# gpauloski/BERT-PyTorch

Measured on AMD Instinct MI355X. Metric: sequences/sec, higher is better.
Workload: dtype bf16; 1 GPU; model=bert_large_uncased_config (24L/1024H/16h, vocab 30528), phase=1, global_batch=768, named_global_batch=65536, seq_len=128, local_batch=96, accumulation=8, optimizer=FusedLAMB (HIP multi-tensor) + fp32 masters, weights=bf16 matmul weights + fp32 LN/bias (fp32 LAMB masters), parallelism=dp1

## Files before the change

### bert_pytorch_amd/models/bert.py

```python

from __future__ import annotations

import logging
import math
from typing import Optional

import torch
import torch.nn.functional as F
from torch import nn

from .. import ops
from ..config import BertConfig

logger = logging.getLogger(__name__)


def _autocast_dtype(ref: torch.Tensor) -> torch.dtype:
    if ref.is_cuda and torch.is_autocast_enabled():
        return torch.get_autocast_gpu_dtype()
    return ref.dtype


class LinearActivation(nn.Module):

    def __init__(self, in_features: int, out_features: int, act: str = "gelu"):
        super().__init__()
        self.in_features = in_features
        self.out_features = out_features
        self.act = act
        self.weight = nn.Parameter(torch.empty(out_features, in_features))
        self.bias = nn.Parameter(torch.empty(out_features))
        self.reset_parameters()

    def reset_parameters(self) -> None:
        nn.init.kaiming_uniform_(self.weight, a=math.sqrt(5))
        bound = 1 / math.sqrt(self.in_features)
        nn.init.uniform_(self.bias, -bound, bound)

    def forward(self, x: torch.Tensor) -> torch.Tensor:
        if self.act in ("gelu", "bias_gelu"):
            y = ops.linear_nobias(x, self.weight)
            return ops.fused_bias_gelu(y, self.bias)
        y = F.linear(x, self.weight, self.bias)
        if self.act in ("tanh", "bias_tanh"):
            return torch.tanh(y)
        if self.act == "relu":
            return F.relu(y)
        if self.act == "swish":
            return y * torch.sigmoid(y)
        raise ValueError(f"unsupported activation {self.act!r}")


class BertEmbeddings(nn.Module):

    def __init__(self, config: BertConfig):
        super().__init__()
        self.word_embeddings = nn.Embedding(config.vocab_size, config.hidden_size)
        self.position_embeddings = nn.Embedding(
            config.max_position_embeddings, config.hidden_size
        )
        if config.next_sentence:
            self.token_type_embeddings = nn.Embedding(
                config.type_vocab_size, config.hidden_size
            )
        else:
            self.token_type_embeddings = None
        self.LayerNorm = ops.FusedLayerNorm(config.hidden_size, eps=1e-12)
        self.dropout_prob = config.hidden_dropout_prob

    def forward(
        self, input_ids: torch.Tensor, token_type_ids: Optional[torch.Tensor]
    ) -> torch.Tensor:
        tok_w = (
            self.token_type_embeddings.weight
            if self.token_type_embeddings is not None
            else None
        )
        return ops.fused_embedding_ln_dropout(
            input_ids,
            token_type_ids if tok_w is not None else None,
            self.word_embeddings.weight,
            self.position_embeddings.weight,
            tok_w,
            self.LayerNorm.weight,
            self.LayerNorm.bias,
            self.dropout_prob,
            self.training,
        )


class _PackedQKV(nn.Module):

    def __init__(self, hidden_size: int):
        super().__init__()
        self.hidden_size = hidden_size
        self.qkv_weight = nn.Parameter(torch.empty(3 * hidden_size, hidden_size))
        self.qkv_bias = nn.Parameter(torch.zeros(3 * hidden_size))

    def forward(self, x: torch.Tensor) -> torch.Tensor:
        return ops.fused_linear(x, self.qkv_weight, self.qkv_bias)

    def _save_to_state_dict(self, destination, prefix, keep_vars):
        h = self.hidden_size
        w = self.qkv_weight if keep_vars else self.qkv_weight.detach()
        b = self.qkv_bias if keep_vars else self.qkv_bias.detach()
        for i, name in enumerate(("query", "key", "value")):
            destination[f"{prefix}{name}.weight"] = w[i * h : (i + 1) * h]
            destination[f"{prefix}{name}.bias"] = b[i * h : (i + 1) * h]

    def _load_from_state_dict(
        self, state_dict, prefix, local_metadata, strict,
        missing_keys, unexpected_keys, error_msgs,
    ):
        h = self.hidden_size
        parts_w, parts_b = [], []
        for name in ("query", "key", "value"):
            wk, bk = f"{prefix}{name}.weight", f"{prefix}{name}.bias"
            if wk in state_dict:
                parts_w.append(state_dict.pop(wk))
            elif strict:
                missing_keys.append(wk)
            if bk in state_dict:
                parts_b.append(state_dict.pop(bk))
            elif strict:
                missing_keys.append(bk)
        with torch.no_grad():
            if len(parts_w) == 3:
                self.qkv_weight.copy_(torch.cat([p.reshape(h, h) for p in parts_w], 0))
            if len(parts_b) == 3:
                self.qkv_bias.copy_(torch.cat([p.reshape(h) for p in parts_b], 0))


class BertSelfOutput(nn.Module):

    def __init__(self, config: BertConfig):
        super().__init__()
        self.dense = nn.Linear(config.hidden_size, config.hidden_size)
        self.LayerNorm = ops.FusedLayerNorm(config.hidden_size, eps=1e-12)
        self.dropout_prob = config.hidden_dropout_prob

    def forward(self, hidden: torch.Tensor, residual: torch.Tensor) -> torch.Tensor:
        y = ops.linear_nobias(hidden, self.dense.weight)
        return ops.fused_bias_dropout_residual_ln(
            y, self.dense.bias, residual,
            self.LayerNorm.weight, self.LayerNorm.bias,
            self.dropout_prob, self.training,
        )


class BertAttention(nn.Module):

    def __init__(self, config: BertConfig):
        super().__init__()
        if config.hidden_size % config.num_attention_heads != 0:
            raise ValueError(
                f"hidden_size {config.hidden_size} not divisible by "
                f"num_attention_heads {config.num_attention_heads}"
            )
        self.num_heads = config.num_attention_heads
        self.self = _PackedQKV(config.hidden_size)
        self.output = BertSelfOutput(config)
        self.dropout_prob = config.attention_probs_dropout_prob

    def forward(
        self, x: torch.Tensor, seqlens: torch.Tensor, max_seqlen: int = 0
    ) -> torch.Tensor:
        qkv = self.self(x)
        if max_seqlen:
            ctx = ops.fused_attention_varlen(
                qkv, seqlens, max_seqlen, self.num_heads,
                self.dropout_prob, self.training,
            )
        else:
            ctx = ops.fused_attention(
                qkv, seqlens, self.num_heads, self.dropout_prob, self.training
            )
        return self.output(ctx, x)


class BertIntermediate(nn.Module):
    def __init__(self, config: BertConfig):
        super().__init__()
        self.dense_act = LinearActivation(
            config.hidden_size, config.intermediate_size, act=config.hidden_act
        )

    def forward(self, x: torch.Tensor) -> torch.Tensor:
        return self.dense_act(x)


class BertOutput(nn.Module):
    def __init__(self, config: BertConfig):
        super().__init__()
        self.dense = nn.Linear(config.intermediate_size, config.hidden_size)
        self.LayerNorm = ops.FusedLayerNorm(config.hidden_size, eps=1e-12)
        self.dropout_prob = config.hidden_dropout_prob

    def forward(self, hidden: torch.Tensor, residual: torch.Tensor) -> torch.Tensor:
        y = ops.linear_nobias(hidden, self.dense.weight)
        return ops.fused_bias_dropout_residual_ln(
            y, self.dense.bias, residual,
            self.LayerNorm.weight, self.LayerNorm.bias,
            self.dropout_prob, self.training,
        )


class BertLayer(nn.Module):
    def __init__(self, config: BertConfig):
        super().__init__()
        self.attention = BertAttention(config)
        self.intermediate = BertIntermediate(config)
        self.output = BertOutput(config)
        self._ffn_gelu = config.hidden_act in ("gelu", "bias_gelu")

    def forward(
        self, x: torch.Tensor, seqlens: torch.Tensor, max_seqlen: int = 0
    ) -> torch.Tensor:
        attn = self.attention(x, seqlens, max_seqlen)
        if self._ffn_gelu and ops.ffn_supported(attn):
            y = ops.fused_ffn(
                attn,
                self.intermediate.dense_act.weight,
                self.intermediate.dense_act.bias,
                self.output.dense.weight,
            )
            return ops.fused_bias_dropout_residual_ln(
                y, self.output.dense.bias, attn,
                self.output.LayerNorm.weight, self.output.LayerNorm.bias,
                self.output.dropout_prob, self.training,
            )
        inter = self.intermediate(attn)
        return self.output(inter, attn)


class BertEncoder(nn.Module):

    def __init__(self, config: BertConfig):
        super().__init__()
        self.layer = nn.ModuleList(
            BertLayer(config) for _ in range(config.num_hidden_layers)
        )
        self.output_all_encoded_layers = config.output_all_encoded_layers
        self._checkpoint_activations = False

    def _checkpointed_forward(self, x, seqlens, max_seqlen=0):
        num_layers = len(self.layer)
        chunk = int(math.sqrt(num_layers)) or 1

        def run(start, end):
            def custom(hidden, lens):
                for layer in self.layer[start:end]:
                    hidden = layer(hidden, lens, max_seqlen)
                return hidden

            return custom

        for start in range(0, num_layers, chunk):
            end = min(start + chunk, num_layers)
            x = torch.utils.checkpoint.checkpoint(
                run(start, end), x, seqlens, use_reentrant=False
            )
        return x

    def forward(
        self, x: torch.Tensor, seqlens: torch.Tensor, max_seqlen: int = 0
    ):
        all_layers = []
        if self._checkpoint_activations:
            x = self._checkpointed_forward(x, seqlens, max_seqlen)
        else:
            for layer in self.layer:
                x = layer(x, seqlens, max_seqlen)
                if self.output_all_encoded_layers:
                    all_layers.append(x)
        if not self.output_all_encoded_layers or self._checkpoint_activations:
            all_layers.append(x)
        return all_layers


class BertPooler(nn.Module):
    def __init__(self, config: BertConfig):
        super().__init__()
        self.dense_act = LinearActivation(
            config.hidden_size, config.hidden_size, act="tanh"
        )

    def forward(self, hidden: torch.Tensor) -> torch.Tensor:
        return self.dense_act(hidden[:, 0])


class BertPredictionHeadTransform(nn.Module):
    def __init__(self, config: BertConfig):
        super().__init__()
        self.dense_act = LinearActivation(
            config.hidden_size, config.hidden_size, act=config.hidden_act
        )
        self.LayerNorm = ops.FusedLayerNorm(config.hidden_size, eps=1e-12)

    def forward(self, x: torch.Tensor) -> torch.Tensor:
        return self.LayerNorm(self.dense_act(x))


class BertLMPredictionHead(nn.Module):

    def __init__(self, config: BertConfig, embedding_weights: torch.Tensor):
        super().__init__()
        self.transform = BertPredictionHeadTransform(config)
        self.decoder = nn.Linear(
            embedding_weights.size(1), embedding_weights.size(0), bias=False
        )
        self.decoder.weight = embedding_weights
        self.bias = nn.Parameter(torch.zeros(embedding_weights.size(0)))

    def forward(self, x: torch.Tensor) -> torch.Tensor:
        x = self.transform(x)
        return F.linear(x, self.decoder.weight, self.bias)


class BertPreTrainingHeads(nn.Module):
    def __init__(self, config: BertConfig, embedding_weights: torch.Tensor):
        super().__init__()
        self.predictions = BertLMPredictionHead(config, embedding_weights)
        if config.next_sentence:
            self.seq_relationship = nn.Linear(config.hidden_size, 2)
        else:
            self.seq_relationship = None

    def forward(self, sequence_output, pooled_output):
        prediction_scores = self.predictions(sequence_output)
        if self.seq_relationship is not None and pooled_output is not None:
            return prediction_scores, self.seq_relationship(pooled_output)
        return prediction_scores, None


class BertOnlyMLMHead(nn.Module):
    def __init__(self, config: BertConfig, embedding_weights: torch.Tensor):
        super().__init__()
        self.predictions = BertLMPredictionHead(config, embedding_weights)

    def forward(self, sequence_output):
        return self.predictions(sequence_output)


class BertOnlyNSPHead(nn.Module):
    def __init__(self, config: BertConfig):
        super().__init__()
        self.seq_relationship = nn.Linear(config.hidden_size, 2)

    def forward(self, pooled_output):
        return self.seq_relationship(pooled_output)


class BertPreTrainedModel(nn.Module):

    def __init__(self, config: BertConfig):
        super().__init__()
        if not isinstance(config, BertConfig):
            raise ValueError("config must be a BertConfig")
        self.config = config

    def init_bert_weights(self, module: nn.Module) -> None:
        if isinstance(module, (nn.Linear, nn.Embedding)):
            module.weight.data.normal_(mean=0.0, std=self.config.initializer_range)
        elif isinstance(module, (LinearActivation,)):
            module.weight.data.normal_(mean=0.0, std=self.config.initializer_range)
        elif isinstance(module, _PackedQKV):
            module.qkv_weight.data.normal_(
                mean=0.0, std=self.config.initializer_range
            )
        elif isinstance(module, ops.FusedLayerNorm):
            module.weight.data.fill_(1.0)
            module.bias.data.zero_()
        if isinstance(module, (nn.Linear, LinearActivation)) and module.bias is not None:
            module.bias.data.zero_()

    def apply_init(self) -> None:
        self.apply(self.init_bert_weights)

    def checkpoint_activations(self, flag: bool) -> None:
        for module in self.modules():
            if isinstance(module, BertEncoder):
                module._checkpoint_activations = flag

    def unpad_inputs(self, flag: bool) -> None:
        for module in self.modules():
            if isinstance(module, BertModel):
                module._unpad_inputs = bool(flag)

    @classmethod
    def from_pretrained(
        cls,
        path: str,
        config: Optional[BertConfig] = None,
        from_tf: bool = False,
        **kw,
    ):
        import os

        if config is None:
            cfg_file = os.path.join(path, "config.json")
            if os.path.isfile(cfg_file):
                config = BertConfig.from_json_file(cfg_file)
            else:
                raise ValueError("config required when path is not a model dir")
        model = cls(config, **kw)
        if from_tf or os.path.isfile(path + ".index"):
            from .tf_import import load_tf_weights

            return load_tf_weights(model, path, strict=False)
        sd_file = path
        if os.path.isdir(path):
            sd_file = os.path.join(path, "pytorch_model.bin")
        state = torch.load(sd_file, map_location="cpu", weights_only=False)
        if isinstance(state, dict) and "model" in state:
            state = state["model"]
        state = {k.removeprefix("module."): v for k, v in state.items()}
        missing, unexpected = model.load_state_dict(state, strict=False)
        if missing:
            logger.info("from_pretrained: missing keys %s", missing)
        if unexpected:
            logger.info("from_pretrained: unexpected keys %s", unexpected)
        return model


class BertModel(BertPreTrainedModel):

    def __init__(self, config: BertConfig):
        super().__init__(config)
        self.embeddings = BertEmbeddings(config)
        self.encoder = BertEncoder(config)
        self.pooler = BertPooler(config) if config.next_sentence else None
        self.output_all_encoded_layers = config.output_all_encoded_layers
        self._unpad_inputs = False
        self.apply_init()

    def forward(
        self,
        input_ids: torch.Tensor,
        token_type_ids: Optional[torch.Tensor] = None,
        attention_mask: Optional[torch.Tensor] = None,
    ):
        if attention_mask is None:
            attention_mask = torch.ones_like(input_ids)
        if token_type_ids is None and self.embeddings.token_type_embeddings is not None:
            token_type_ids = torch.zeros_like(input_ids)
        seqlens = attention_mask.sum(dim=-1, dtype=torch.int32)

        emb = self.embeddings(input_ids, token_type_ids)
        if self._unpad_inputs:
            encoded_layers = self._unpadded_encoder(emb, attention_mask)
        else:
            encoded_layers = self.encoder(emb, seqlens)
        sequence_output = encoded_layers[-1]
        pooled = self.pooler(sequence_output) if self.pooler is not None else None
        if not self.output_all_encoded_layers:
            encoded_layers = encoded_layers[-1]
        return encoded_layers, pooled


    def _unpadded_encoder(self, emb: torch.Tensor, attention_mask: torch.Tensor):
        bsz, seq, hidden = emb.shape
        dest, cu_seqlens, _total, t_pad = ops.unpad_index(attention_mask)
        packed = ops.pack_rows(emb.reshape(bsz * seq, hidden), dest, t_pad)
        layers = self.encoder(packed, cu_seqlens, seq)
        return [
            ops.unpack_rows(y, dest, bsz * seq).view(bsz, seq, hidden)
            for y in layers
        ]


class BertForPreTraining(BertPreTrainedModel):

    def __init__(self, config: BertConfig):
        super().__init__(config)
        self.bert = BertModel(config)
        self.cls = BertPreTrainingHeads(
            config, self.bert.embeddings.word_embeddings.weight
        )
        for m in (self.cls,):
            m.apply(self.init_bert_weights)
        self.cls.predictions.decoder.weight = (
            self.bert.embeddings.word_embeddings.weight
        )

    def forward(
        self,
        input_ids,
        token_type_ids=None,
        attention_mask=None,
        masked_lm_labels=None,
        max_predictions_per_seq=None,
        compute_mlm_loss=False,
    ):
        encoded, pooled = self.bert(input_ids, token_type_ids, attention_mask)
        sequence_output = encoded[-1] if isinstance(encoded, list) else encoded
        if masked_lm_labels is None:
            return self.cls(sequence_output, pooled)
        flat_labels = masked_lm_labels.reshape(-1)
        if max_predictions_per_seq is not None:
            num = flat_labels.numel()
            cap = masked_lm_labels.shape[0] * max_predictions_per_seq
            mask = flat_labels != -1
            slots = torch.cumsum(mask.to(torch.long), 0) - 1
            slots = torch.where(
                mask, slots.clamp_(max=cap), torch.full_like(slots, cap)
            )
            positions = torch.zeros(
                cap + 1, dtype=torch.long, device=flat_labels.device
            )
            positions.scatter_(
                0, slots, torch.arange(num, device=flat_labels.device)
            )
            gathered_labels = torch.full(
                (cap + 1,), -1, dtype=flat_labels.dtype,
                device=flat_labels.device,
            )
            gathered_labels.scatter_(0, slots, flat_labels)
            positions = positions[:cap]
            gathered_labels = gathered_labels[:cap]
        else:
            positions = torch.nonzero(
                flat_labels != -1, as_tuple=False
            ).squeeze(-1)
            gathered_labels = flat_labels.index_select(0, positions)
        hidden = sequence_output.reshape(-1, sequence_output.shape[-1])
        masked_hidden = hidden.index_select(0, positions)
        if compute_mlm_loss:
            head = self.cls.predictions
            scores = ops.mlm_decoder_loss(
                head.transform(masked_hidden),
                head.decoder.weight,
                head.bias,
                gathered_labels,
            )
        else:
            scores = self.cls.predictions(masked_hidden)
        seq_rel = (
            self.cls.seq_relationship(pooled)
            if self.cls.seq_relationship is not None and pooled is not None
            else None
        )
        return scores, seq_rel, gathered_labels


class BertForMaskedLM(BertPreTrainedModel):
    def __init__(self, config: BertConfig):
        super().__init__(config)
        self.bert = BertModel(config)
        self.cls = BertOnlyMLMHead(
            config, self.bert.embeddings.word_embeddings.weight
        )
        self.cls.apply(self.init_bert_weights)
        self.cls.predictions.decoder.weight = (
            self.bert.embeddings.word_embeddings.weight
        )

    def forward(
        self, input_ids, token_type_ids=None, attention_mask=None,
        masked_lm_labels=None,
    ):
        encoded, _ = self.bert(input_ids, token_type_ids, attention_mask)
        seq_out = encoded[-1] if isinstance(encoded, list) else encoded
        scores = self.cls(seq_out)
        if masked_lm_labels is not None:
            return ops.fused_cross_entropy(
                scores.view(-1, scores.shape[-1]), masked_lm_labels.view(-1), -1
            )
        return scores


class BertForNextSentencePrediction(BertPreTrainedModel):
    def __init__(self, config: BertConfig):
        super().__init__(config)
        self.bert = BertModel(config)
        self.cls = BertOnlyNSPHead(config)
        self.cls.apply(self.init_bert_weights)

    def forward(
        self, input_ids, token_type_ids=None, attention_mask=None,
        next_sentence_label=None,
    ):
        _, pooled = self.bert(input_ids, token_type_ids, attention_mask)
        score = self.cls(pooled)
        if next_sentence_label is not None:
            return F.cross_entropy(
                score.view(-1, 2), next_sentence_label.view(-1), ignore_index=-1
            )
        return score


class BertForSequenceClassification(BertPreTrainedModel):
    def __init__(self, config: BertConfig, num_labels: int = 2):
        super().__init__(config)
        self.num_labels = num_labels
        self.bert = BertModel(config)
        self.dropout = nn.Dropout(config.hidden_dropout_prob)
        self.classifier = nn.Linear(config.hidden_size, num_labels)
        self.classifier.apply(self.init_bert_weights)

    def forward(self, input_ids, token_type_ids=None, attention_mask=None, labels=None):
        _, pooled = self.bert(input_ids, token_type_ids, attention_mask)
        logits = self.classifier(self.dropout(pooled))
        if labels is not None:
            return F.cross_entropy(logits.view(-1, self.num_labels), labels.view(-1))
        return logits


class BertForMultipleChoice(BertPreTrainedModel):
    def __init__(self, config: BertConfig, num_choices: int = 2):
        super().__init__(config)
        self.num_choices = num_choices
        self.bert = BertModel(config)
        self.dropout = nn.Dropout(config.hidden_dropout_prob)
        self.classifier = nn.Linear(config.hidden_size, 1)
        self.classifier.apply(self.init_bert_weights)

    def forward(self, input_ids, token_type_ids=None, attention_mask=None, labels=None):
        flat = lambda t: t.view(-1, t.size(-1)) if t is not None else None
        _, pooled = self.bert(flat(input_ids), flat(token_type_ids), flat(attention_mask))
        logits = self.classifier(self.dropout(pooled)).view(-1, self.num_choices)
        if labels is not None:
            return F.cross_entropy(logits, labels)
        return logits


class BertForTokenClassification(BertPreTrainedModel):

    def __init__(self, config: BertConfig, num_labels: int = 2):
        super().__init__(config)
        self.num_labels = num_labels
        self.bert = BertModel(config)
        self.dropout = nn.Dropout(config.hidden_dropout_prob)
        self.classifier = nn.Linear(config.hidden_size, num_labels)
        self.classifier.apply(self.init_bert_weights)

    def forward(self, input_ids, token_type_ids=None, attention_mask=None, labels=None):
        encoded, _ = self.bert(input_ids, token_type_ids, attention_mask)
        seq_out = encoded[-1] if isinstance(encoded, list) else encoded
        logits = self.classifier(self.dropout(seq_out))
        if labels is not None:
            if attention_mask is not None:
                active = attention_mask.view(-1) == 1
                return F.cross_entropy(
                    logits.view(-1, self.num_labels)[active],
                    labels.view(-1)[active],
                )
            return F.cross_entropy(logits.view(-1, self.num_labels), labels.view(-1))
        return logits


class BertForQuestionAnswering(BertPreTrainedModel):

    def __init__(self, config: BertConfig):
        super().__init__(config)
        self.bert = BertModel(config)
        self.qa_outputs = nn.Linear(config.hidden_size, 2)
        self.qa_outputs.apply(self.init_bert_weights)

    def forward(self, input_ids, token_type_ids=None, attention_mask=None):
        encoded, _ = self.bert(input_ids, token_type_ids, attention_mask)
        seq_out = encoded[-1] if isinstance(encoded, list) else encoded
        logits = self.qa_outputs(seq_out)
        start_logits, end_logits = logits.split(1, dim=-1)
        return start_logits.squeeze(-1), end_logits.squeeze(-1)
```

### bert_pytorch_amd/ops/fused_residual.py

```python

from __future__ import annotations

from typing import Optional

import torch

from . import _reference, extension, use_native
from .rng import next_philox


class _FusedBiasDropoutResidualLN(torch.autograd.Function):
    @staticmethod
    def forward(ctx, x, bias, residual, weight, ln_bias, p, training, eps):
        ext = extension()
        x2d = x.contiguous().view(-1, x.shape[-1])
        r2d = residual.contiguous().view(-1, x.shape[-1])
        seed, offset = next_philox(x2d.numel()) if (training and p > 0) else (0, 0)
        y, z, mask, mean, rstd = ext.bias_dropout_residual_ln_fwd(
            x2d, bias, r2d, weight, ln_bias, p if training else 0.0, eps, seed, offset
        )
        ctx.save_for_backward(z, mask, weight, mean, rstd)
        ctx.p = p if training else 0.0
        ctx.has_bias = bias is not None
        ctx.shape = x.shape
        return y.view(x.shape)

    @staticmethod
    def backward(ctx, dy):
        ext = extension()
        z, mask, weight, mean, rstd = ctx.saved_tensors
        dy2d = dy.contiguous().view(-1, dy.shape[-1])
        dx, dbias, dz, dw, db = ext.bias_dropout_residual_ln_bwd(
            dy2d, z, mask, weight, mean, rstd, ctx.p, ctx.has_bias
        )
        return (
            dx.view(ctx.shape),
            dbias if ctx.has_bias else None,
            dz.view(ctx.shape),
            dw,
            db,
            None,
            None,
            None,
        )


def fused_bias_dropout_residual_ln(
    x: torch.Tensor,
    bias: Optional[torch.Tensor],
    residual: torch.Tensor,
    weight: torch.Tensor,
    ln_bias: torch.Tensor,
    p: float,
    training: bool,
    eps: float = 1e-12,
) -> torch.Tensor:
    if use_native(x):
        return _FusedBiasDropoutResidualLN.apply(
            x, bias, residual, weight, ln_bias, p, training, eps
        )
    return _reference.bias_dropout_residual_ln(
        x, bias, residual, weight, ln_bias, p, training, eps
    )
```

### csrc/bind.cpp

```cpp
#include <torch/extension.h>

#include "ops.h"

PYBIND11_MODULE(TORCH_EXTENSION_NAME, m) {
  m.doc() = "bert_pytorch_amd gfx950 HIP kernels";
  m.def("ln_fwd", &bpa::ln_fwd, "fused LayerNorm forward");
  m.def("ln_bwd", &bpa::ln_bwd, "fused LayerNorm backward");
  m.def("bias_gelu_fwd", &bpa::bias_gelu_fwd);
  m.def("bias_gelu_bwd", &bpa::bias_gelu_bwd);
  m.def("col_sum", &bpa::col_sum, "column sum [rows,H] -> fp32 [H]");
  m.def("gemm_bias_gelu_fwd", &bpa::gemm_bias_gelu_fwd,
        "hipblaslt GEMM with fused bias+GELU epilogue (+aux)");
  m.def("gemm_dgelu_bgrad", &bpa::gemm_dgelu_bgrad,
        "hipblaslt dgrad GEMM with fused dGELU+bias-grad epilogue");
  m.def("gemm_gelu_aux_supported", &bpa::gemm_gelu_aux_supported);
  m.def("bias_dropout_residual_ln_fwd", &bpa::bias_dropout_residual_ln_fwd);
  m.def("bias_dropout_residual_ln_bwd", &bpa::bias_dropout_residual_ln_bwd);
  m.def("embedding_ln_dropout_fwd", &bpa::embedding_ln_dropout_fwd);
  m.def("embedding_ln_dropout_bwd", &bpa::embedding_ln_dropout_bwd);
  m.def("ce_fwd", &bpa::ce_fwd);
  m.def("ce_bwd", &bpa::ce_bwd);
  m.def("attention_fwd", &bpa::attention_fwd);
  m.def("attention_bwd", &bpa::attention_bwd);
  m.def("attention_varlen_fwd", &bpa::attention_varlen_fwd,
        "packed [T_pad,3H] attention over a cu_seqlens index");
  m.def("attention_varlen_bwd", &bpa::attention_varlen_bwd);
  m.def("pack_rows", &bpa::pack_rows,
        "[B*S,H] -> [T_pad,H]: row i to row dest[i], dest<0 dropped");
  m.def("unpack_rows", &bpa::unpack_rows,
        "[T_pad,H] -> [B*S,H]: inverse of pack_rows, dropped rows zero");
  m.def("tr16_probe", &bpa::tr16_probe);
  m.def("wgrad_tn", &bpa::wgrad_tn, py::arg("dy"), py::arg("x"),
        py::arg("splitk_override") = 0);
  m.def("wgrad_tn_supported", &bpa::wgrad_tn_supported);
  m.def("mlm_head_fwd", &bpa::mlm_head_fwd,
        "MFMA MLM-decoder GEMM with fused bias + CE-forward epilogue");
  m.def("mlm_head_supported", &bpa::mlm_head_supported);
  m.def("wgrad_tn_profitable", &bpa::wgrad_tn_profitable);
  m.def("multi_tensor_l2norm_sq", &bpa::multi_tensor_l2norm_sq);
  m.def("multi_tensor_clip_scale", &bpa::multi_tensor_clip_scale);
  m.def("fused_lamb", &bpa::fused_lamb);
  m.def("fused_adam", &bpa::fused_adam);
  m.def("tok_create_wordpiece", &bpa_tok::create_wordpiece);
  m.def("tok_encode_wordpiece", &bpa_tok::encode_wordpiece);
  m.def("tok_create_bpe", &bpa_tok::create_bpe);
  m.def("tok_encode_bpe", &bpa_tok::encode_bpe);
  m.def("tok_train_bpe", &bpa_tok::train_bpe);
}
```

### csrc/ops.h

```cpp
#pragma once

#include <cstdint>
#include <string>
#include <utility>
#include <vector>

namespace bpa_tok {
int64_t create_wordpiece(std::vector<std::string> vocab, std::string unk);
std::pair<std::vector<std::string>, std::vector<int64_t>> encode_wordpiece(
    int64_t handle, std::vector<std::string> words);
int64_t create_bpe(std::vector<std::string> vocab,
                   std::vector<std::string> merge_lines);
std::pair<std::vector<std::string>, std::vector<int64_t>> encode_bpe(
    int64_t handle, std::vector<std::string> pretokens);
std::vector<std::string> train_bpe(std::vector<std::string> words,
                                   std::vector<int64_t> counts,
                                   int64_t num_merges);
}

#ifndef BPA_TOK_ONLY
#include <torch/extension.h>

namespace bpa {

std::vector<torch::Tensor> ln_fwd(torch::Tensor x, torch::Tensor gamma,
                                  torch::Tensor beta, double eps);
std::vector<torch::Tensor> ln_bwd(torch::Tensor dy, torch::Tensor x,
                                  torch::Tensor gamma, torch::Tensor mean,
                                  torch::Tensor rstd);
torch::Tensor bias_gelu_fwd(torch::Tensor x, torch::Tensor bias);
std::vector<torch::Tensor> bias_gelu_bwd(torch::Tensor dy, torch::Tensor x,
                                         torch::Tensor bias);
torch::Tensor col_sum(torch::Tensor x);
torch::Tensor col_reduce_full(torch::Tensor parts);
torch::Tensor col_stats(torch::Tensor dy, torch::Tensor z,
                        torch::Tensor dx_src, torch::Tensor mean,
                        torch::Tensor rstd);
std::vector<torch::Tensor> gemm_bias_gelu_fwd(torch::Tensor x,
                                              torch::Tensor w1,
                                              torch::Tensor b1);
std::vector<torch::Tensor> gemm_dgelu_bgrad(torch::Tensor dout,
                                            torch::Tensor w2,
                                            torch::Tensor aux);
bool gemm_gelu_aux_supported();
std::vector<torch::Tensor> bias_dropout_residual_ln_fwd(
    torch::Tensor x, c10::optional<torch::Tensor> bias, torch::Tensor residual,
    torch::Tensor gamma, torch::Tensor beta, double p, double eps,
    int64_t seed, int64_t offset);
std::vector<torch::Tensor> bias_dropout_residual_ln_bwd(
    torch::Tensor dy, torch::Tensor z, torch::Tensor mask, torch::Tensor gamma,
    torch::Tensor mean, torch::Tensor rstd, double p, bool has_bias);
std::vector<torch::Tensor> embedding_ln_dropout_fwd(
    torch::Tensor ids, c10::optional<torch::Tensor> tt, torch::Tensor word,
    torch::Tensor pos, c10::optional<torch::Tensor> tok, torch::Tensor gamma,
    torch::Tensor beta, double p, double eps, int64_t seed, int64_t offset,
    torch::ScalarType out_dtype);
std::vector<torch::Tensor> embedding_ln_dropout_bwd(
    torch::Tensor dy, torch::Tensor ids, c10::optional<torch::Tensor> tt,
    torch::Tensor z, torch::Tensor mask, torch::Tensor gamma,
    torch::Tensor mean, torch::Tensor rstd, double p, int64_t vocab,
    int64_t max_pos, int64_t n_types);
std::vector<torch::Tensor> ce_fwd(torch::Tensor logits, torch::Tensor labels,
                                  int64_t ignore_index);
torch::Tensor ce_bwd(torch::Tensor dloss, torch::Tensor logits,
                     torch::Tensor labels, torch::Tensor lse,
                     torch::Tensor count, int64_t ignore_index);
std::vector<torch::Tensor> attention_fwd(torch::Tensor qkv,
                                         torch::Tensor seqlens,
                                         int64_t num_heads, double p,
                                         int64_t seed, int64_t offset);
torch::Tensor tr16_probe(int64_t addr_mode);
torch::Tensor wgrad_tn(torch::Tensor dy, torch::Tensor x,
                       int64_t splitk_override);
std::vector<torch::Tensor> mlm_head_fwd(torch::Tensor h, torch::Tensor w,
                                        torch::Tensor bias,
                                        torch::Tensor labels,
                                        int64_t ignore_index);
bool mlm_head_supported(int64_t P, int64_t V, int64_t K);
bool wgrad_tn_supported(int64_t K, int64_t M, int64_t N);
bool wgrad_tn_profitable(int64_t K, int64_t M, int64_t N);
torch::Tensor attention_bwd(torch::Tensor dout, torch::Tensor qkv,
                            torch::Tensor seqlens, torch::Tensor out,
                            torch::Tensor lse, torch::Tensor dmask,
                            int64_t num_heads, double p, int64_t seed,
                            int64_t offset);
std::vector<torch::Tensor> attention_varlen_fwd(
    torch::Tensor qkv, torch::Tensor cu_seqlens, int64_t max_seqlen,
    int64_t num_heads, double p, int64_t seed, int64_t offset);
torch::Tensor attention_varlen_bwd(torch::Tensor dout, torch::Tensor qkv,
                                   torch::Tensor cu_seqlens,
                                   int64_t max_seqlen, torch::Tensor out,
                                   torch::Tensor lse, torch::Tensor dmask,
                                   int64_t num_heads, double p,
                                   int64_t seed, int64_t offset);
torch::Tensor pack_rows(torch::Tensor x, torch::Tensor dest, int64_t t_pad);
torch::Tensor unpack_rows(torch::Tensor y, torch::Tensor dest,
                          int64_t padded_rows);
torch::Tensor multi_tensor_l2norm_sq(std::vector<torch::Tensor> tensors);
void multi_tensor_clip_scale(std::vector<torch::Tensor> grads,
                             torch::Tensor gnorm_sq, double max_norm);
void fused_lamb(std::vector<torch::Tensor> params,
                std::vector<torch::Tensor> grads,
                std::vector<torch::Tensor> ms, std::vector<torch::Tensor> vs,
                torch::Tensor gnorm_sq, double lr, double beta1, double beta2,
                double eps, double wd, int64_t step, bool bias_correction,
                bool grad_averaging, double max_grad_norm, bool use_ratio);
void fused_adam(std::vector<torch::Tensor> params,
                std::vector<torch::Tensor> grads,
                std::vector<torch::Tensor> ms, std::vector<torch::Tensor> vs,
                double lr, double beta1, double beta2, double eps, double wd,
                int64_t step, bool bias_correction, bool adam_w);

}

#endif
```

### csrc/ops/fused_residual.hip

```cpp

#include <torch/extension.h>
#include <ATen/hip/HIPContext.h>

#include "../checks.h"
#include "../ops.h"
#include "rowwise.h"

namespace bpa {

template <typename T, int VEC, int ITEMS, bool HAS_BIAS, bool TRAIN_DROP>
__global__ void bdrl_fwd_kernel(
    const T* __restrict__ x, const float* __restrict__ bias,
    const T* __restrict__ residual, const float* __restrict__ gamma,
    const float* __restrict__ beta, T* __restrict__ y, T* __restrict__ z,
    uint8_t* __restrict__ mask, float* __restrict__ mean,
    float* __restrict__ rstd, int rows, int H, float p, float eps,
    uint64_t seed, uint64_t offset) {
  __shared__ float red[16], red2[16];
  const int row = blockIdx.x;
  if (row >= rows) return;
  const int64_t base = static_cast<int64_t>(row) * H;
  const float keep_scale = TRAIN_DROP ? 1.0f / (1.0f - p) : 1.0f;
  Philox philox(seed);

  float zv[ITEMS][VEC];
  int cols[ITEMS];
  float sum = 0.f;
#pragma unroll
  for (int i = 0; i < ITEMS; ++i) {
    const int c = (i * blockDim.x + threadIdx.x) * VEC;
    cols[i] = c;
    if (c < H) {
      T xv[VEC], rv[VEC], zt[VEC];
      load_slice(x + base + c, xv);
      load_slice(residual + base + c, rv);
      uint8_t mv[VEC];
      if (TRAIN_DROP) keep_mask(philox, offset, base + c, p, mv);
#pragma unroll
      for (int k = 0; k < VEC; ++k) {
        float t = DTraits<T>::to_f32(xv[k]);
        if (HAS_BIAS) t += bias[c + k];
        if (TRAIN_DROP) t = mv[k] ? t * keep_scale : 0.f;
        t += DTraits<T>::to_f32(rv[k]);
        zv[i][k] = t;
        zt[k] = DTraits<T>::from_f32(t);
        sum += t;
      }
      store_slice(z + base + c, zt);
      if (TRAIN_DROP) store_mask(mask + base + c, mv);
    }
  }
  const RowStats st =
      ln_row_stats(zv, cols, sum, H, eps, red, red2, mean, rstd, row);
  ln_affine_store<T, VEC, ITEMS>(zv, cols, st, gamma, beta, y + base, H);
}

template <typename T, int VEC, int ITEMS, bool TRAIN_DROP>
__global__ void bdrl_bwd_dx_kernel(
    const T* __restrict__ dy, const T* __restrict__ z,
    const uint8_t* __restrict__ mask, const float* __restrict__ gamma,
    const float* __restrict__ mean, const float* __restrict__ rstd,
    T* __restrict__ dx, T* __restrict__ dz_res, int rows, int H, float p) {
  __shared__ float red[32];
  const int row = blockIdx.x;
  if (row >= rows) return;
  const int64_t base = static_cast<int64_t>(row) * H;
  const float mu = mean[row], rs = rstd[row];
  const float keep_scale = TRAIN_DROP ? 1.0f / (1.0f - p) : 1.0f;

  float dw[ITEMS][VEC], zh[ITEMS][VEC];
  uint8_t mv[ITEMS][VEC];
  int cols[ITEMS];
  float s1 = 0.f, s2 = 0.f;
#pragma unroll
  for (int i = 0; i < ITEMS; ++i) {
    const int c = (i * blockDim.x + threadIdx.x) * VEC;
    cols[i] = c;
    if (c < H) {
      T dt[VEC], zt[VEC];
      load_slice(dy + base + c, dt);
      load_slice(z + base + c, zt);
      if (TRAIN_DROP) load_mask(mask + base + c, mv[i]);
#pragma unroll
      for (int k = 0; k < VEC; ++k)
        ln_bwd_elem(zt[k], dt[k], &gamma[c + k], mu, rs, dw[i][k], zh[i][k],
                    s1, s2);
    }
  }
  ln_bwd_row_means(s1, s2, H, red);
#pragma unroll
  for (int i = 0; i < ITEMS; ++i) {
    const int c = cols[i];
    if (c < H) {
      T dzo[VEC], dxo[VEC];
#pragma unroll
      for (int k = 0; k < VEC; ++k) {
        const float dzk = ln_bwd_dz(dw[i][k], zh[i][k], rs, s1, s2);
        dzo[k] = DTraits<T>::from_f32(dzk);
        const float dxk =
            TRAIN_DROP ? (mv[i][k] ? dzk * keep_scale : 0.f) : dzk;
        dxo[k] = DTraits<T>::from_f32(dxk);
      }
      store_slice(dz_res + base + c, dzo);
      store_slice(dx + base + c, dxo);
    }
  }
}

std::vector<torch::Tensor> bias_dropout_residual_ln_fwd(
    torch::Tensor x, c10::optional<torch::Tensor> bias, torch::Tensor residual,
    torch::Tensor gamma, torch::Tensor beta, double p, double eps,
    int64_t seed, int64_t offset) {
  TORCH_CHECK(x.dim() == 2 && x.is_contiguous(), "bdrl_fwd: bad x");
  const int rows = x.size(0), H = x.size(1);
  auto res_c = residual.contiguous();
  TORCH_CHECK(res_c.scalar_type() == x.scalar_type(),
              "bdrl_fwd: residual dtype must match x");
  auto gamma_f = gamma.contiguous().to(torch::kFloat32);
  auto beta_f = beta.contiguous().to(torch::kFloat32);
  torch::Tensor bias_f;
  const bool has_bias = bias.has_value();
  if (has_bias) bias_f = bias->contiguous().to(torch::kFloat32);
  const bool train_drop = p > 0.0;

  auto y = torch::empty_like(x);
  auto z = torch::empty_like(x);
  auto fopts = x.options().dtype(torch::kFloat32);
  auto mask = train_drop
                  ? torch::empty({rows, H}, x.options().dtype(torch::kUInt8))
                  : torch::empty({0}, x.options().dtype(torch::kUInt8));
  auto mean = torch::empty({rows}, fopts);
  auto rstd = torch::empty({rows}, fopts);
  auto stream = at::hip::getCurrentHIPStream();
  DISPATCH_ROW_DTYPE(x.scalar_type(), "bdrl_fwd", [&] {
    TORCH_CHECK(H % kVec == 0, "bdrl_fwd: H % ", kVec, " != 0");
    launch_by_items("bdrl_fwd", H / kVec, [&](auto items_c, int threads) {
      by_flag(has_bias, [&](auto has_bias_c) {
        by_flag(train_drop, [&](auto train_c) {
          hipLaunchKernelGGL(
              (bdrl_fwd_kernel<scalar_t, kVec, decltype(items_c)::value,
                               decltype(has_bias_c)::value,
                               decltype(train_c)::value>),
              dim3(rows), dim3(threads), 0, stream, dptr<scalar_t>(x),
              has_bias ? bias_f.data_ptr<float>() : nullptr,
              dptr<scalar_t>(res_c), gamma_f.data_ptr<float>(),
              beta_f.data_ptr<float>(), dptr<scalar_t>(y), dptr<scalar_t>(z),
              train_drop ? mask.data_ptr<uint8_t>() : nullptr,
              mean.data_ptr<float>(), rstd.data_ptr<float>(), rows, H,
              static_cast<float>(p), static_cast<float>(eps),
              static_cast<uint64_t>(seed), static_cast<uint64_t>(offset));
        });
      });
    });
  });
  return {y, z, mask, mean, rstd};
}

std::vector<torch::Tensor> bias_dropout_residual_ln_bwd(
    torch::Tensor dy, torch::Tensor z, torch::Tensor mask, torch::Tensor gamma,
    torch::Tensor mean, torch::Tensor rstd, double p, bool has_bias) {
  check_rows_2d("bdrl_bwd", "z", z);
  check_like("bdrl_bwd", "dy", dy, "z", z);
  const int rows = z.size(0), H = z.size(1);
  check_row_stat("bdrl_bwd", "mean", mean, rows);
  check_row_stat("bdrl_bwd", "rstd", rstd, rows);
  check_param("bdrl_bwd", "gamma", gamma, H);
  if (p > 0.0) check_drop_mask("bdrl_bwd", mask, rows, H);
  auto gamma_f = gamma.contiguous().to(torch::kFloat32);
  auto dx = torch::empty_like(z);
  auto dz_res = torch::empty_like(z);
  auto fopts = z.options().dtype(torch::kFloat32);
  const bool train_drop = p > 0.0;
  auto stream = at::hip::getCurrentHIPStream();
  DISPATCH_ROW_DTYPE(z.scalar_type(), "bdrl_bwd", [&] {
    TORCH_CHECK(H % kVec == 0, "bdrl_bwd: H % ", kVec, " != 0");
    launch_by_items("bdrl_bwd", H / kVec, [&](auto items_c, int threads) {
      by_flag(train_drop, [&](auto train_c) {
        hipLaunchKernelGGL(
            (bdrl_bwd_dx_kernel<scalar_t, kVec, decltype(items_c)::value,
                                decltype(train_c)::value>),
            dim3(rows), dim3(threads), 0, stream, dptr<scalar_t>(dy),
            dptr<scalar_t>(z), train_drop ? mask.data_ptr<uint8_t>() : nullptr,
            gamma_f.data_ptr<float>(), mean.data_ptr<float>(),
            rstd.data_ptr<float>(), dptr<scalar_t>(dx),
            dptr<scalar_t>(dz_res), rows, H, static_cast<float>(p));
      });
    });
  });
  auto out = col_stats(dy, z, has_bias ? dx : torch::Tensor(), mean, rstd);
  auto dgamma = out.narrow(0, 0, H).contiguous();
  auto dbeta = out.narrow(0, H, H).contiguous();
  auto dbias =
      has_bias ? out.narrow(0, 2 * H, H).contiguous() : torch::empty({0}, fopts);
  if (gamma.scalar_type() != torch::kFloat32) {
    dgamma = dgamma.to(gamma.scalar_type());
    dbeta = dbeta.to(gamma.scalar_type());
    if (has_bias) dbias = dbias.to(gamma.scalar_type());
  }
  return {dx, dbias, dz_res, dgamma, dbeta};
}

}
```

### csrc/ops/layernorm.hip

```cpp

#include <torch/extension.h>
#include <ATen/hip/HIPContext.h>

#include "../checks.h"
#include "../ops.h"
#include "rowwise.h"

namespace bpa {

template <typename T, int VEC, int ITEMS>
__global__ void ln_fwd_kernel(const T* __restrict__ x,
                              const float* __restrict__ gamma,
                              const float* __restrict__ beta,
                              T* __restrict__ y, float* __restrict__ mean,
                              float* __restrict__ rstd, int rows, int H,
                              float eps) {
  __shared__ float red[16], red2[16];
  const int row = blockIdx.x;
  if (row >= rows) return;
  const int64_t base = static_cast<int64_t>(row) * H;

  float v[ITEMS][VEC];
  int cols[ITEMS];
  float sum = 0.f;
#pragma unroll
  for (int i = 0; i < ITEMS; ++i) {
    const int c = (i * blockDim.x + threadIdx.x) * VEC;
    cols[i] = c;
    if (c < H) {
      T t[VEC];
      load_slice(x + base + c, t);
#pragma unroll
      for (int k = 0; k < VEC; ++k) {
        v[i][k] = DTraits<T>::to_f32(t[k]);
        sum += v[i][k];
      }
    }
  }
  const RowStats st =
      ln_row_stats(v, cols, sum, H, eps, red, red2, mean, rstd, row);
  ln_affine_store<T, VEC, ITEMS>(v, cols, st, gamma, beta, y + base, H);
}

template <typename T, int VEC, int ITEMS>
__global__ void ln_bwd_dx_kernel(const T* __restrict__ dy,
                                 const T* __restrict__ x,
                                 const float* __restrict__ gamma,
                                 const float* __restrict__ mean,
                                 const float* __restrict__ rstd,
                                 T* __restrict__ dx, int rows, int H) {
  __shared__ float red[32];
  const int row = blockIdx.x;
  if (row >= rows) return;
  const int64_t base = static_cast<int64_t>(row) * H;
  const float mu = mean[row], rs = rstd[row];

  float dw[ITEMS][VEC], xh[ITEMS][VEC];
  int cols[ITEMS];
  float s1 = 0.f, s2 = 0.f;
#pragma unroll
  for (int i = 0; i < ITEMS; ++i) {
    const int c = (i * blockDim.x + threadIdx.x) * VEC;
    cols[i] = c;
    if (c < H) {
      T dt[VEC], xt[VEC];
      load_slice(dy + base + c, dt);
      load_slice(x + base + c, xt);
#pragma unroll
      for (int k = 0; k < VEC; ++k)
        ln_bwd_elem(xt[k], dt[k], &gamma[c + k], mu, rs, dw[i][k], xh[i][k],
                    s1, s2);
    }
  }
  ln_bwd_row_means(s1, s2, H, red);
#pragma unroll
  for (int i = 0; i < ITEMS; ++i) {
    const int c = cols[i];
    if (c < H) {
      T o[VEC];
#pragma unroll
      for (int k = 0; k < VEC; ++k)
        o[k] = DTraits<T>::from_f32(
            ln_bwd_dz(dw[i][k], xh[i][k], rs, s1, s2));
      store_slice(dx + base + c, o);
    }
  }
}

template <typename T, int VEC, bool HAS_BIAS>
__global__ void col_stats_kernel(const T* __restrict__ dy,
                                 const T* __restrict__ z,
                                 const T* __restrict__ dx_src,
                                 const float* __restrict__ mean,
                                 const float* __restrict__ rstd,
                                 float* __restrict__ part, int rows, int H,
                                 int rows_per_chunk) {
  const int c = (blockIdx.x * blockDim.x + threadIdx.x) * VEC;
  if (c >= H) return;
  const int r0 = blockIdx.y * rows_per_chunk;
  const int r1 = min(r0 + rows_per_chunk, rows);
  float acc_g[VEC] = {}, acc_b[VEC] = {}, acc_bias[VEC] = {};
  for (int r = r0; r < r1; ++r) {
    const int64_t base = static_cast<int64_t>(r) * H + c;
    const float mu = mean[r], rs = rstd[r];
    T dt[VEC], zt[VEC], xt[VEC];
    *reinterpret_cast<uint4*>(dt) = *reinterpret_cast<const uint4*>(dy + base);
    *reinterpret_cast<uint4*>(zt) = *reinterpret_cast<const uint4*>(z + base);
    if (HAS_BIAS)
      *reinterpret_cast<uint4*>(xt) =
          *reinterpret_cast<const uint4*>(dx_src + base);
#pragma unroll
    for (int k = 0; k < VEC; ++k) {
      const float d = DTraits<T>::to_f32(dt[k]);
      acc_g[k] += d * (DTraits<T>::to_f32(zt[k]) - mu) * rs;
      acc_b[k] += d;
      if (HAS_BIAS) acc_bias[k] += DTraits<T>::to_f32(xt[k]);
    }
  }
  const int nsl = HAS_BIAS ? 3 : 2;
  float* p = part + static_cast<int64_t>(blockIdx.y) * nsl * H + c;
#pragma unroll
  for (int k = 0; k < VEC; ++k) {
    p[k] = acc_g[k];
    p[H + k] = acc_b[k];
    if (HAS_BIAS) p[2 * H + k] = acc_bias[k];
  }
}

__global__ void col_reduce_blocked_kernel(const float* __restrict__ parts,
                                          int nparts, int S, int rows_per_j,
                                          float* __restrict__ out) {
  const int c = (blockIdx.x * blockDim.x + threadIdx.x) * 4;
  if (c >= S) return;
  const int p0 = blockIdx.y * rows_per_j;
  const int p1 = min(p0 + rows_per_j, nparts);
  float acc[4] = {};
  for (int p = p0; p < p1; ++p) {
    const float* src = parts + static_cast<int64_t>(p) * S + c;
    if (c + 4 <= S) {
      float v[4];
      *reinterpret_cast<uint4*>(v) = *reinterpret_cast<const uint4*>(src);
#pragma unroll
      for (int k = 0; k < 4; ++k) acc[k] += v[k];
    } else {
      for (int k = 0; c + k < S; ++k) acc[k] += src[k];
    }
  }
  float* dst = out + static_cast<int64_t>(blockIdx.y) * S + c;
  for (int k = 0; k < 4 && c + k < S; ++k) dst[k] = acc[k];
}

__global__ void col_reduce_ordered_kernel(const float* __restrict__ parts,
                                          int nparts, int S, int chunk,
                                          float* __restrict__ tmp,
                                          unsigned int* __restrict__ counters,
                                          float* __restrict__ out) {
  const int c = (blockIdx.x * blockDim.x + threadIdx.x) * 4;
  const bool active = c < S;
  if (active) {
    const int p0 = blockIdx.y * chunk;
    const int p1 = min(p0 + chunk, nparts);
    float acc[4] = {};
    for (int p = p0; p < p1; ++p) {
      const float* src = parts + static_cast<int64_t>(p) * S + c;
      if (c + 4 <= S) {
        float v[4];
        *reinterpret_cast<uint4*>(v) = *reinterpret_cast<const uint4*>(src);
#pragma unroll
        for (int k = 0; k < 4; ++k) acc[k] += v[k];
      } else {
        for (int k = 0; c + k < S; ++k) acc[k] += src[k];
      }
    }
    float* dst = tmp + static_cast<int64_t>(blockIdx.y) * S + c;
    for (int k = 0; k < 4 && c + k < S; ++k) dst[k] = acc[k];
  }
  __threadfence();
  __shared__ bool is_last;
  __syncthreads();
  if (threadIdx.x == 0)
    is_last = atomicAdd(&counters[blockIdx.x], 1u) == gridDim.y - 1;
  __syncthreads();
  if (!is_last || !active) return;
  __threadfence();
  constexpr int kFoldBatch = 16;
  const int ny = static_cast<int>(gridDim.y);
  const int nk = min(4, S - c);
  float sum[4] = {};
  for (int j0 = 0; j0 < ny; j0 += kFoldBatch) {
    float v[kFoldBatch][4];
#pragma unroll
    for (int u = 0; u < kFoldBatch; ++u) {
      const int j = min(j0 + u, ny - 1);
      const float* src = tmp + static_cast<int64_t>(j) * S + c;
      if (nk == 4) {
        *reinterpret_cast<uint4*>(v[u]) =
            *reinterpret_cast<const uint4*>(src);
      } else {
#pragma unroll
        for (int k = 0; k < 4; ++k) v[u][k] = k < nk ? src[k] : 0.f;
      }
    }
#pragma unroll
    for (int u = 0; u < kFoldBatch; ++u)
      if (j0 + u < ny) {
        for (int k = 0; k < 4; ++k) sum[k] += v[u][k];
      }
  }
  for (int k = 0; k < nk; ++k) out[c + k] = sum[k];
}

constexpr int kColChunk = 32;

torch::Tensor col_reduce_full(torch::Tensor parts) {
  const int nparts = parts.size(0);
  const int S = parts.size(1);
  auto stream = at::hip::getCurrentHIPStream();
  const int xblocks = (S / 4 + 255) / 256;
  if (nparts <= 48) {
    auto out = torch::empty({S}, parts.options());
    hipLaunchKernelGGL(col_reduce_blocked_kernel, dim3(xblocks, 1),
                       dim3(256), 0, stream, parts.data_ptr<float>(), nparts,
                       S, nparts, out.data_ptr<float>());
    return out;
  }
  const int chunk = kColChunk;
  const int yblocks = (nparts + chunk - 1) / chunk;
  auto out = torch::empty({S}, parts.options());
  auto tmp = torch::empty({yblocks, S}, parts.options());
  auto counters = torch::zeros({xblocks}, parts.options().dtype(torch::kInt32));
  dim3 grid(xblocks, yblocks);
  hipLaunchKernelGGL(col_reduce_ordered_kernel, grid, dim3(256), 0, stream,
                     parts.data_ptr<float>(), nparts, S, chunk,
                     tmp.data_ptr<float>(),
                     reinterpret_cast<unsigned int*>(counters.data_ptr<int>()),
                     out.data_ptr<float>());
  return out;
}

torch::Tensor col_stats(torch::Tensor dy, torch::Tensor z,
                        torch::Tensor dx_src, torch::Tensor mean,
                        torch::Tensor rstd) {
  const int rows = z.size(0), H = z.size(1);
  const int rows_per_chunk = 16;
  const int n_chunks = (rows + rows_per_chunk - 1) / rows_per_chunk;
  const bool has_bias = dx_src.defined();
  auto part = torch::empty({n_chunks, (has_bias ? 3 : 2) * H},
                           z.options().dtype(torch::kFloat32));
  auto stream = at::hip::getCurrentHIPStream();
  DISPATCH_ROW_DTYPE(z.scalar_type(), "col_stats", [&] {
    const int threads = tmin(256, ((H / kVec + 63) / 64) * 64);
    dim3 grid((H / kVec + threads - 1) / threads, n_chunks);
    by_flag(has_bias, [&](auto bias_c) {
      hipLaunchKernelGGL(
          (col_stats_kernel<scalar_t, kVec, decltype(bias_c)::value>), grid,
          dim3(threads), 0, stream, dptr<scalar_t>(dy), dptr<scalar_t>(z),
          has_bias ? dptr<scalar_t>(dx_src) : nullptr, mean.data_ptr<float>(),
          rstd.data_ptr<float>(), part.data_ptr<float>(), rows, H,
          rows_per_chunk);
    });
  });
  return col_reduce_full(part);
}

std::vector<torch::Tensor> ln_fwd(torch::Tensor x, torch::Tensor gamma,
                                  torch::Tensor beta, double eps) {
  TORCH_CHECK(x.dim() == 2 && x.is_contiguous(), "ln_fwd: x must be 2D contiguous");
  const int rows = x.size(0), H = x.size(1);
  auto gamma_f = gamma.contiguous().to(torch::kFloat32);
  auto beta_f = beta.contiguous().to(torch::kFloat32);
  auto y = torch::empty_like(x);
  auto opts = x.options().dtype(torch::kFloat32);
  auto mean = torch::empty({rows}, opts);
  auto rstd = torch::empty({rows}, opts);
  auto stream = at::hip::getCurrentHIPStream();
  DISPATCH_ROW_DTYPE(x.scalar_type(), "ln_fwd", [&] {
    TORCH_CHECK(H % kVec == 0, "ln_fwd: H must be a multiple of ", kVec);
    launch_by_items("ln_fwd", H / kVec, [&](auto items_c, int threads) {
      hipLaunchKernelGGL(
          (ln_fwd_kernel<scalar_t, kVec, decltype(items_c)::value>),
          dim3(rows), dim3(threads), 0, stream, dptr<scalar_t>(x),
          gamma_f.data_ptr<float>(), beta_f.data_ptr<float>(),
          dptr<scalar_t>(y), mean.data_ptr<float>(), rstd.data_ptr<float>(),
          rows, H, static_cast<float>(eps));
    });
  });
  return {y, mean, rstd};
}

std::vector<torch::Tensor> ln_bwd(torch::Tensor dy, torch::Tensor x,
                                  torch::Tensor gamma, torch::Tensor mean,
                                  torch::Tensor rstd) {
  check_rows_2d("ln_bwd", "x", x);
  check_like("ln_bwd", "dy", dy, "x", x);
  const int rows = x.size(0), H = x.size(1);
  check_row_stat("ln_bwd", "mean", mean, rows);
  check_row_stat("ln_bwd", "rstd", rstd, rows);
  check_param("ln_bwd", "gamma", gamma, H);
  auto gamma_f = gamma.contiguous().to(torch::kFloat32);
  auto dx = torch::empty_like(x);
  auto stream = at::hip::getCurrentHIPStream();
  DISPATCH_ROW_DTYPE(x.scalar_type(), "ln_bwd", [&] {
    TORCH_CHECK(H % kVec == 0, "ln_bwd: H must be a multiple of ", kVec);
    launch_by_items("ln_bwd", H / kVec, [&](auto items_c, int threads) {
      hipLaunchKernelGGL(
          (ln_bwd_dx_kernel<scalar_t, kVec, decltype(items_c)::value>),
          dim3(rows), dim3(threads), 0, stream, dptr<scalar_t>(dy),
          dptr<scalar_t>(x), gamma_f.data_ptr<float>(),
          mean.data_ptr<float>(), rstd.data_ptr<float>(), dptr<scalar_t>(dx),
          rows, H);
    });
  });
  auto dgb = col_stats(dy, x, torch::Tensor(), mean, rstd);
  auto dgamma = dgb.narrow(0, 0, H);
  auto dbeta = dgb.narrow(0, H, H);
  if (gamma.scalar_type() != torch::kFloat32) {
    return {dx, dgamma.to(gamma.scalar_type()), dbeta.to(gamma.scalar_type())};
  }
  return {dx, dgamma.contiguous(), dbeta.contiguous()};
}

}
```

### csrc/ops/rowwise.h

```cpp
#pragma once

#include <torch/extension.h>

#include <type_traits>

#include "../common.h"

#define DISPATCH_ROW_DTYPE(TYPE, NAME, ...)                                  \
  [&] {                                                                      \
    if (TYPE == at::kBFloat16) {                                             \
      using scalar_t = __hip_bfloat16;                                       \
      constexpr int kVec = 8;                                                \
      return __VA_ARGS__();                                                  \
    } else if (TYPE == at::kHalf) {                                          \
      using scalar_t = __half;                                               \
      constexpr int kVec = 8;                                                \
      return __VA_ARGS__();                                                  \
    } else if (TYPE == at::kFloat) {                                         \
      using scalar_t = float;                                                \
      constexpr int kVec = 4;                                                \
      return __VA_ARGS__();                                                  \
    } else {                                                                 \
      TORCH_CHECK(false, NAME, ": unsupported dtype");                       \
    }                                                                        \
  }()

namespace bpa {

template <typename T>
inline T* dptr(const torch::Tensor& t) {
  return reinterpret_cast<T*>(t.data_ptr());
}

template <typename LaunchFn>
inline void launch_by_items(const char* op, int slices, LaunchFn&& fn) {
  if (slices <= 256) {
    fn(std::integral_constant<int, 1>{}, ((slices + 63) / 64) * 64);
  } else if (slices <= 512) {
    fn(std::integral_constant<int, 2>{}, 256);
  } else if (slices <= 1024) {
    fn(std::integral_constant<int, 2>{}, 512);
  } else if (slices <= 2048) {
    fn(std::integral_constant<int, 4>{}, 512);
  } else {
    TORCH_CHECK(slices <= 4096, op, ": H too large");
    fn(std::integral_constant<int, 4>{}, 1024);
  }
}

template <typename Fn>
inline void by_flag(bool flag, Fn&& fn) {
  if (flag) fn(std::true_type{});
  else fn(std::false_type{});
}

template <typename T, int VEC>
__device__ __forceinline__ void load_slice(const T* p, T (&t)[VEC]) {
  if (sizeof(T) * VEC == 16) {
    *reinterpret_cast<uint4*>(t) = *reinterpret_cast<const uint4*>(p);
  } else {
#pragma unroll
    for (int k = 0; k < VEC; ++k) t[k] = p[k];
  }
}

template <typename T, int VEC>
__device__ __forceinline__ void store_slice(T* p, const T (&t)[VEC]) {
  if (sizeof(T) * VEC == 16) {
    *reinterpret_cast<uint4*>(p) = *reinterpret_cast<const uint4*>(t);
  } else {
#pragma unroll
    for (int k = 0; k < VEC; ++k) p[k] = t[k];
  }
}

template <int VEC>
__device__ __forceinline__ void keep_mask(const Philox& philox,
                                          uint64_t offset, int64_t elem_index,
                                          float p, uint8_t (&mv)[VEC]) {
#pragma unroll
  for (int q = 0; q < VEC / 4; ++q) {
    uint32_t r4[4];
    philox(offset + elem_index / 4 + q, r4);
#pragma unroll
    for (int j = 0; j < 4; ++j)
      mv[q * 4 + j] = u32_to_uniform(r4[j]) >= p ? 1 : 0;
  }
}

template <int VEC>
__device__ __forceinline__ void load_mask(const uint8_t* p,
                                          uint8_t (&mv)[VEC]) {
  using word_t = std::conditional_t<VEC == 8, uint2, uint32_t>;
  *reinterpret_cast<word_t*>(mv) = *reinterpret_cast<const word_t*>(p);
}

template <int VEC>
__device__ __forceinline__ void store_mask(uint8_t* p,
                                           const uint8_t (&mv)[VEC]) {
  using word_t = std::conditional_t<VEC == 8, uint2, uint32_t>;
  *reinterpret_cast<word_t*>(p) = *reinterpret_cast<const word_t*>(mv);
}

struct RowStats {
  float mu, rs;
};

template <int VEC, int ITEMS>
__device__ __forceinline__ RowStats ln_row_stats(
    const float (&v)[ITEMS][VEC], const int (&cols)[ITEMS], float sum, int H,
    float eps, float* red, float* red2, float* mean, float* rstd, int row) {
  const float mu = block_reduce_sum1(sum, red) / H;
  float sq = 0.f;
#pragma unroll
  for (int i = 0; i < ITEMS; ++i) {
    if (cols[i] < H) {
#pragma unroll
      for (int k = 0; k < VEC; ++k) {
        const float d = v[i][k] - mu;
        sq += d * d;
      }
    }
  }
  const float var = block_reduce_sum1(sq, red2) / H;
  const float rs = rsqrtf(var + eps);
  if (threadIdx.x == 0) {
    mean[row] = mu;
    rstd[row] = rs;
  }
  return {mu, rs};
}

__device__ __forceinline__ float ln_affine(float v, RowStats st, float g,
                                           float b) {
  return (v - st.mu) * st.rs * g + b;
}

template <typename T, int VEC, int ITEMS>
__device__ __forceinline__ void ln_affine_store(
    const float (&v)[ITEMS][VEC], const int (&cols)[ITEMS], RowStats st,
    const float* gamma, const float* beta, T* y_row, int H) {
#pragma unroll
  for (int i = 0; i < ITEMS; ++i) {
    const int c = cols[i];
    if (c < H) {
      T o[VEC];
#pragma unroll
      for (int k = 0; k < VEC; ++k)
        o[k] = DTraits<T>::from_f32(
            ln_affine(v[i][k], st, gamma[c + k], beta[c + k]));
      store_slice(y_row + c, o);
    }
  }
}

template <typename T>
__device__ __forceinline__ void ln_bwd_elem(T x, T dy, const float* gamma,
                                            float mu, float rs, float& dw,
                                            float& xh, float& s1, float& s2) {
  xh = (DTraits<T>::to_f32(x) - mu) * rs;
  dw = DTraits<T>::to_f32(dy) * *gamma;
  s1 += dw * xh;
  s2 += dw;
}

__device__ __forceinline__ void ln_bwd_row_means(float& s1, float& s2, int H,
                                                 float* red) {
  block_reduce_sum2(s1, s2, red);
  s1 /= H;
  s2 /= H;
}

__device__ __forceinline__ float ln_bwd_dz(float dw, float xh, float rs,
                                           float s1, float s2) {
  return rs * (dw - s2 - xh * s1);
}

}
```

Before: 2501 seq/s.

## Fuse LN-backward column reductions and fork residual gradient into junction kernel

```diff
diff --git a/bert_pytorch_amd/models/bert.py b/bert_pytorch_amd/models/bert.py
--- a/bert_pytorch_amd/models/bert.py
+++ b/bert_pytorch_amd/models/bert.py
@@ -139,12 +139,12 @@
         self.LayerNorm = ops.FusedLayerNorm(config.hidden_size, eps=1e-12)
         self.dropout_prob = config.hidden_dropout_prob
 
-    def forward(self, hidden: torch.Tensor, residual: torch.Tensor) -> torch.Tensor:
+    def forward(self, hidden: torch.Tensor, residual: torch.Tensor, fork: bool = False):
         y = ops.linear_nobias(hidden, self.dense.weight)
         return ops.fused_bias_dropout_residual_ln(
             y, self.dense.bias, residual,
             self.LayerNorm.weight, self.LayerNorm.bias,
-            self.dropout_prob, self.training,
+            self.dropout_prob, self.training, fork=fork,
         )
 
 
@@ -163,8 +163,9 @@
         self.dropout_prob = config.attention_probs_dropout_prob
 
     def forward(
-        self, x: torch.Tensor, seqlens: torch.Tensor, max_seqlen: int = 0
-    ) -> torch.Tensor:
+        self, x, seqlens: torch.Tensor, max_seqlen: int = 0, fork: bool = False
+    ):
+        x, x_res = x if isinstance(x, tuple) else (x, x)
         qkv = self.self(x)
         if max_seqlen:
             ctx = ops.fused_attention_varlen(
@@ -175,7 +176,7 @@
             ctx = ops.fused_attention(
                 qkv, seqlens, self.num_heads, self.dropout_prob, self.training
             )
-        return self.output(ctx, x)
+        return self.output(ctx, x_res, fork)
 
 
 class BertIntermediate(nn.Module):
@@ -196,12 +197,12 @@
         self.LayerNorm = ops.FusedLayerNorm(config.hidden_size, eps=1e-12)
         self.dropout_prob = config.hidden_dropout_prob
 
-    def forward(self, hidden: torch.Tensor, residual: torch.Tensor) -> torch.Tensor:
+    def forward(self, hidden: torch.Tensor, residual: torch.Tensor, fork: bool = False):
         y = ops.linear_nobias(hidden, self.dense.weight)
         return ops.fused_bias_dropout_residual_ln(
             y, self.dense.bias, residual,
             self.LayerNorm.weight, self.LayerNorm.bias,
-            self.dropout_prob, self.training,
+            self.dropout_prob, self.training, fork=fork,
         )
 
 
@@ -214,9 +215,9 @@
         self._ffn_gelu = config.hidden_act in ("gelu", "bias_gelu")
 
     def forward(
-        self, x: torch.Tensor, seqlens: torch.Tensor, max_seqlen: int = 0
-    ) -> torch.Tensor:
-        attn = self.attention(x, seqlens, max_seqlen)
+        self, x, seqlens: torch.Tensor, max_seqlen: int = 0, fork: bool = False
+    ):
+        attn, attn_res = self.attention(x, seqlens, max_seqlen, fork=True)
         if self._ffn_gelu and ops.ffn_supported(attn):
             y = ops.fused_ffn(
                 attn,
@@ -225,12 +226,12 @@
                 self.output.dense.weight,
             )
             return ops.fused_bias_dropout_residual_ln(
-                y, self.output.dense.bias, attn,
+                y, self.output.dense.bias, attn_res,
                 self.output.LayerNorm.weight, self.output.LayerNorm.bias,
-                self.output.dropout_prob, self.training,
+                self.output.dropout_prob, self.training, fork=fork,
             )
         inter = self.intermediate(attn)
-        return self.output(inter, attn)
+        return self.output(inter, attn_res, fork)
 
 
 class BertEncoder(nn.Module):
@@ -249,8 +250,9 @@
 
         def run(start, end):
             def custom(hidden, lens):
-                for layer in self.layer[start:end]:
-                    hidden = layer(hidden, lens, max_seqlen)
+                for i in range(start, end):
+                    hidden = self.layer[i](hidden, lens, max_seqlen,
+                                           fork=i + 1 < end)
                 return hidden
 
             return custom
@@ -269,10 +271,11 @@
         if self._checkpoint_activations:
             x = self._checkpointed_forward(x, seqlens, max_seqlen)
         else:
-            for layer in self.layer:
-                x = layer(x, seqlens, max_seqlen)
+            last = len(self.layer) - 1
+            for i, layer in enumerate(self.layer):
+                x = layer(x, seqlens, max_seqlen, fork=i < last)
                 if self.output_all_encoded_layers:
-                    all_layers.append(x)
+                    all_layers.append(x[0] if i < last else x)
         if not self.output_all_encoded_layers or self._checkpoint_activations:
             all_layers.append(x)
         return all_layers
diff --git a/bert_pytorch_amd/ops/fused_residual.py b/bert_pytorch_amd/ops/fused_residual.py
--- a/bert_pytorch_amd/ops/fused_residual.py
+++ b/bert_pytorch_amd/ops/fused_residual.py
@@ -1,7 +1,8 @@
 
 from __future__ import annotations
 
-from typing import Optional
+import os
+from typing import Optional, Tuple, Union
 
 import torch
 
@@ -11,7 +12,8 @@
 
 class _FusedBiasDropoutResidualLN(torch.autograd.Function):
     @staticmethod
-    def forward(ctx, x, bias, residual, weight, ln_bias, p, training, eps):
+    def forward(ctx, x, bias, residual, weight, ln_bias, p, training, eps,
+                fork):
         ext = extension()
         x2d = x.contiguous().view(-1, x.shape[-1])
         r2d = residual.contiguous().view(-1, x.shape[-1])
@@ -23,15 +25,25 @@
         ctx.p = p if training else 0.0
         ctx.has_bias = bias is not None
         ctx.shape = x.shape
-        return y.view(x.shape)
+        y = y.view(x.shape)
+        if not fork:
+            return y
+        ctx.set_materialize_grads(False)
+        return y, y.detach()
 
     @staticmethod
-    def backward(ctx, dy):
+    def backward(ctx, dy, dy_fork=None):
         ext = extension()
         z, mask, weight, mean, rstd = ctx.saved_tensors
+        if dy is None:
+            dy, dy_fork = dy_fork, None
+        if dy is None:
+            return (None,) * 9
         dy2d = dy.contiguous().view(-1, dy.shape[-1])
+        if dy_fork is not None:
+            dy_fork = dy_fork.contiguous().view(-1, dy.shape[-1])
         dx, dbias, dz, dw, db = ext.bias_dropout_residual_ln_bwd(
-            dy2d, z, mask, weight, mean, rstd, ctx.p, ctx.has_bias
+            dy2d, z, mask, weight, mean, rstd, ctx.p, ctx.has_bias, dy_fork
         )
         return (
             dx.view(ctx.shape),
@@ -39,6 +51,7 @@
             dz.view(ctx.shape),
             dw,
             db,
+            None,
             None,
             None,
             None,
@@ -54,11 +67,18 @@
     p: float,
     training: bool,
     eps: float = 1e-12,
-) -> torch.Tensor:
+    fork: bool = False,
+) -> Union[torch.Tensor, Tuple[torch.Tensor, torch.Tensor]]:
     if use_native(x):
-        return _FusedBiasDropoutResidualLN.apply(
-            x, bias, residual, weight, ln_bias, p, training, eps
+        if fork and os.environ.get("BPA_JUNCTION_FORK") != "0":
+            return _FusedBiasDropoutResidualLN.apply(
+                x, bias, residual, weight, ln_bias, p, training, eps, True
+            )
+        y = _FusedBiasDropoutResidualLN.apply(
+            x, bias, residual, weight, ln_bias, p, training, eps, False
         )
-    return _reference.bias_dropout_residual_ln(
+        return (y, y) if fork else y
+    y = _reference.bias_dropout_residual_ln(
         x, bias, residual, weight, ln_bias, p, training, eps
     )
+    return (y, y.view_as(y)) if fork else y
diff --git a/csrc/bind.cpp b/csrc/bind.cpp
--- a/csrc/bind.cpp
+++ b/csrc/bind.cpp
@@ -15,7 +15,10 @@
         "hipblaslt dgrad GEMM with fused dGELU+bias-grad epilogue");
   m.def("gemm_gelu_aux_supported", &bpa::gemm_gelu_aux_supported);
   m.def("bias_dropout_residual_ln_fwd", &bpa::bias_dropout_residual_ln_fwd);
-  m.def("bias_dropout_residual_ln_bwd", &bpa::bias_dropout_residual_ln_bwd);
+  m.def("bias_dropout_residual_ln_bwd", &bpa::bias_dropout_residual_ln_bwd,
+        py::arg("dy"), py::arg("z"), py::arg("mask"), py::arg("gamma"),
+        py::arg("mean"), py::arg("rstd"), py::arg("p"), py::arg("has_bias"),
+        py::arg("dy2") = py::none());
   m.def("embedding_ln_dropout_fwd", &bpa::embedding_ln_dropout_fwd);
   m.def("embedding_ln_dropout_bwd", &bpa::embedding_ln_dropout_bwd);
   m.def("ce_fwd", &bpa::ce_fwd);
diff --git a/csrc/ops.h b/csrc/ops.h
--- a/csrc/ops.h
+++ b/csrc/ops.h
@@ -33,9 +33,6 @@
                                          torch::Tensor bias);
 torch::Tensor col_sum(torch::Tensor x);
 torch::Tensor col_reduce_full(torch::Tensor parts);
-torch::Tensor col_stats(torch::Tensor dy, torch::Tensor z,
-                        torch::Tensor dx_src, torch::Tensor mean,
-                        torch::Tensor rstd);
 std::vector<torch::Tensor> gemm_bias_gelu_fwd(torch::Tensor x,
                                               torch::Tensor w1,
                                               torch::Tensor b1);
@@ -49,7 +46,8 @@
     int64_t seed, int64_t offset);
 std::vector<torch::Tensor> bias_dropout_residual_ln_bwd(
     torch::Tensor dy, torch::Tensor z, torch::Tensor mask, torch::Tensor gamma,
-    torch::Tensor mean, torch::Tensor rstd, double p, bool has_bias);
+    torch::Tensor mean, torch::Tensor rstd, double p, bool has_bias,
+    c10::optional<torch::Tensor> dy2);
 std::vector<torch::Tensor> embedding_ln_dropout_fwd(
     torch::Tensor ids, c10::optional<torch::Tensor> tt, torch::Tensor word,
     torch::Tensor pos, c10::optional<torch::Tensor> tok, torch::Tensor gamma,
diff --git a/csrc/ops/fused_residual.hip b/csrc/ops/fused_residual.hip
--- a/csrc/ops/fused_residual.hip
+++ b/csrc/ops/fused_residual.hip
@@ -55,58 +55,6 @@
   ln_affine_store<T, VEC, ITEMS>(zv, cols, st, gamma, beta, y + base, H);
 }
 
-template <typename T, int VEC, int ITEMS, bool TRAIN_DROP>
-__global__ void bdrl_bwd_dx_kernel(
-    const T* __restrict__ dy, const T* __restrict__ z,
-    const uint8_t* __restrict__ mask, const float* __restrict__ gamma,
-    const float* __restrict__ mean, const float* __restrict__ rstd,
-    T* __restrict__ dx, T* __restrict__ dz_res, int rows, int H, float p) {
-  __shared__ float red[32];
-  const int row = blockIdx.x;
-  if (row >= rows) return;
-  const int64_t base = static_cast<int64_t>(row) * H;
-  const float mu = mean[row], rs = rstd[row];
-  const float keep_scale = TRAIN_DROP ? 1.0f / (1.0f - p) : 1.0f;
-
-  float dw[ITEMS][VEC], zh[ITEMS][VEC];
-  uint8_t mv[ITEMS][VEC];
-  int cols[ITEMS];
-  float s1 = 0.f, s2 = 0.f;
-#pragma unroll
-  for (int i = 0; i < ITEMS; ++i) {
-    const int c = (i * blockDim.x + threadIdx.x) * VEC;
-    cols[i] = c;
-    if (c < H) {
-      T dt[VEC], zt[VEC];
-      load_slice(dy + base + c, dt);
-      load_slice(z + base + c, zt);
-      if (TRAIN_DROP) load_mask(mask + base + c, mv[i]);
-#pragma unroll
-      for (int k = 0; k < VEC; ++k)
-        ln_bwd_elem(zt[k], dt[k], &gamma[c + k], mu, rs, dw[i][k], zh[i][k],
-                    s1, s2);
-    }
-  }
-  ln_bwd_row_means(s1, s2, H, red);
-#pragma unroll
-  for (int i = 0; i < ITEMS; ++i) {
-    const int c = cols[i];
-    if (c < H) {
-      T dzo[VEC], dxo[VEC];
-#pragma unroll
-      for (int k = 0; k < VEC; ++k) {
-        const float dzk = ln_bwd_dz(dw[i][k], zh[i][k], rs, s1, s2);
-        dzo[k] = DTraits<T>::from_f32(dzk);
-        const float dxk =
-            TRAIN_DROP ? (mv[i][k] ? dzk * keep_scale : 0.f) : dzk;
-        dxo[k] = DTraits<T>::from_f32(dxk);
-      }
-      store_slice(dz_res + base + c, dzo);
-      store_slice(dx + base + c, dxo);
-    }
-  }
-}
-
 std::vector<torch::Tensor> bias_dropout_residual_ln_fwd(
     torch::Tensor x, c10::optional<torch::Tensor> bias, torch::Tensor residual,
     torch::Tensor gamma, torch::Tensor beta, double p, double eps,
@@ -158,9 +106,15 @@
 
 std::vector<torch::Tensor> bias_dropout_residual_ln_bwd(
     torch::Tensor dy, torch::Tensor z, torch::Tensor mask, torch::Tensor gamma,
-    torch::Tensor mean, torch::Tensor rstd, double p, bool has_bias) {
+    torch::Tensor mean, torch::Tensor rstd, double p, bool has_bias,
+    c10::optional<torch::Tensor> dy2) {
   check_rows_2d("bdrl_bwd", "z", z);
   check_like("bdrl_bwd", "dy", dy, "z", z);
+  if (dy2.has_value()) {
+    TORCH_CHECK(dy2->device() == z.device(), "bdrl_bwd: dy2 device ",
+                dy2->device(), " does not match z device ", z.device());
+    check_like("bdrl_bwd", "dy2", *dy2, "z", z);
+  }
   const int rows = z.size(0), H = z.size(1);
   check_row_stat("bdrl_bwd", "mean", mean, rows);
   check_row_stat("bdrl_bwd", "rstd", rstd, rows);
@@ -170,24 +124,15 @@
   auto dx = torch::empty_like(z);
   auto dz_res = torch::empty_like(z);
   auto fopts = z.options().dtype(torch::kFloat32);
-  const bool train_drop = p > 0.0;
   auto stream = at::hip::getCurrentHIPStream();
+  torch::Tensor part;
   DISPATCH_ROW_DTYPE(z.scalar_type(), "bdrl_bwd", [&] {
     TORCH_CHECK(H % kVec == 0, "bdrl_bwd: H % ", kVec, " != 0");
-    launch_by_items("bdrl_bwd", H / kVec, [&](auto items_c, int threads) {
-      by_flag(train_drop, [&](auto train_c) {
-        hipLaunchKernelGGL(
-            (bdrl_bwd_dx_kernel<scalar_t, kVec, decltype(items_c)::value,
-                                decltype(train_c)::value>),
-            dim3(rows), dim3(threads), 0, stream, dptr<scalar_t>(dy),
-            dptr<scalar_t>(z), train_drop ? mask.data_ptr<uint8_t>() : nullptr,
-            gamma_f.data_ptr<float>(), mean.data_ptr<float>(),
-            rstd.data_ptr<float>(), dptr<scalar_t>(dx),
-            dptr<scalar_t>(dz_res), rows, H, static_cast<float>(p));
-      });
-    });
+    part = ln_bwd_rows<scalar_t, kVec, true>(
+        "bdrl_bwd", dy, dy2.has_value() ? *dy2 : torch::Tensor(), z, mask,
+        gamma_f, mean, rstd, dx, dz_res, p, has_bias, stream);
   });
-  auto out = col_stats(dy, z, has_bias ? dx : torch::Tensor(), mean, rstd);
+  auto out = col_reduce_full(part);
   auto dgamma = out.narrow(0, 0, H).contiguous();
   auto dbeta = out.narrow(0, H, H).contiguous();
   auto dbias =
diff --git a/csrc/ops/layernorm.hip b/csrc/ops/layernorm.hip
--- a/csrc/ops/layernorm.hip
+++ b/csrc/ops/layernorm.hip
@@ -42,88 +42,30 @@
   ln_affine_store<T, VEC, ITEMS>(v, cols, st, gamma, beta, y + base, H);
 }
 
-template <typename T, int VEC, int ITEMS>
-__global__ void ln_bwd_dx_kernel(const T* __restrict__ dy,
-                                 const T* __restrict__ x,
-                                 const float* __restrict__ gamma,
-                                 const float* __restrict__ mean,
-                                 const float* __restrict__ rstd,
-                                 T* __restrict__ dx, int rows, int H) {
-  __shared__ float red[32];
-  const int row = blockIdx.x;
-  if (row >= rows) return;
-  const int64_t base = static_cast<int64_t>(row) * H;
-  const float mu = mean[row], rs = rstd[row];
+constexpr int kStripBatch = 16;
 
-  float dw[ITEMS][VEC], xh[ITEMS][VEC];
-  int cols[ITEMS];
-  float s1 = 0.f, s2 = 0.f;
+__device__ __forceinline__ void strip_sum(const float* __restrict__ m, int r0,
+                                          int r1, int S, int c, int nk,
+                                          float (&sum)[4]) {
+  for (int j0 = r0; j0 < r1; j0 += kStripBatch) {
+    float v[kStripBatch][4];
 #pragma unroll
-  for (int i = 0; i < ITEMS; ++i) {
-    const int c = (i * blockDim.x + threadIdx.x) * VEC;
-    cols[i] = c;
-    if (c < H) {
-      T dt[VEC], xt[VEC];
-      load_slice(dy + base + c, dt);
-      load_slice(x + base + c, xt);
+    for (int u = 0; u < kStripBatch; ++u) {
+      const int j = min(j0 + u, r1 - 1);
+      const float* src = m + static_cast<int64_t>(j) * S + c;
+      if (nk == 4) {
+        *reinterpret_cast<uint4*>(v[u]) =
+            *reinterpret_cast<const uint4*>(src);
+      } else {
 #pragma unroll
-      for (int k = 0; k < VEC; ++k)
-        ln_bwd_elem(xt[k], dt[k], &gamma[c + k], mu, rs, dw[i][k], xh[i][k],
-                    s1, s2);
+        for (int k = 0; k < 4; ++k) v[u][k] = k < nk ? src[k] : 0.f;
+      }
     }
-  }
-  ln_bwd_row_means(s1, s2, H, red);
 #pragma unroll
-  for (int i = 0; i < ITEMS; ++i) {
-    const int c = cols[i];
-    if (c < H) {
-      T o[VEC];
-#pragma unroll
-      for (int k = 0; k < VEC; ++k)
-        o[k] = DTraits<T>::from_f32(
-            ln_bwd_dz(dw[i][k], xh[i][k], rs, s1, s2));
-      store_slice(dx + base + c, o);
-    }
-  }
-}
-
-template <typename T, int VEC, bool HAS_BIAS>
-__global__ void col_stats_kernel(const T* __restrict__ dy,
-                                 const T* __restrict__ z,
-                                 const T* __restrict__ dx_src,
-                                 const float* __restrict__ mean,
-                                 const float* __restrict__ rstd,
-                                 float* __restrict__ part, int rows, int H,
-                                 int rows_per_chunk) {
-  const int c = (blockIdx.x * blockDim.x + threadIdx.x) * VEC;
-  if (c >= H) return;
-  const int r0 = blockIdx.y * rows_per_chunk;
-  const int r1 = min(r0 + rows_per_chunk, rows);
-  float acc_g[VEC] = {}, acc_b[VEC] = {}, acc_bias[VEC] = {};
-  for (int r = r0; r < r1; ++r) {
-    const int64_t base = static_cast<int64_t>(r) * H + c;
-    const float mu = mean[r], rs = rstd[r];
-    T dt[VEC], zt[VEC], xt[VEC];
-    *reinterpret_cast<uint4*>(dt) = *reinterpret_cast<const uint4*>(dy + base);
-    *reinterpret_cast<uint4*>(zt) = *reinterpret_cast<const uint4*>(z + base);
-    if (HAS_BIAS)
-      *reinterpret_cast<uint4*>(xt) =
-          *reinterpret_cast<const uint4*>(dx_src + base);
-#pragma unroll
-    for (int k = 0; k < VEC; ++k) {
-      const float d = DTraits<T>::to_f32(dt[k]);
-      acc_g[k] += d * (DTraits<T>::to_f32(zt[k]) - mu) * rs;
-      acc_b[k] += d;
-      if (HAS_BIAS) acc_bias[k] += DTraits<T>::to_f32(xt[k]);
-    }
-  }
-  const int nsl = HAS_BIAS ? 3 : 2;
-  float* p = part + static_cast<int64_t>(blockIdx.y) * nsl * H + c;
-#pragma unroll
-  for (int k = 0; k < VEC; ++k) {
-    p[k] = acc_g[k];
-    p[H + k] = acc_b[k];
-    if (HAS_BIAS) p[2 * H + k] = acc_bias[k];
+    for (int u = 0; u < kStripBatch; ++u)
+      if (j0 + u < r1) {
+        for (int k = 0; k < 4; ++k) sum[k] += v[u][k];
+      }
   }
 }
 
@@ -134,20 +76,11 @@
   if (c >= S) return;
   const int p0 = blockIdx.y * rows_per_j;
   const int p1 = min(p0 + rows_per_j, nparts);
+  const int nk = min(4, S - c);
   float acc[4] = {};
-  for (int p = p0; p < p1; ++p) {
-    const float* src = parts + static_cast<int64_t>(p) * S + c;
-    if (c + 4 <= S) {
-      float v[4];
-      *reinterpret_cast<uint4*>(v) = *reinterpret_cast<const uint4*>(src);
-#pragma unroll
-      for (int k = 0; k < 4; ++k) acc[k] += v[k];
-    } else {
-      for (int k = 0; c + k < S; ++k) acc[k] += src[k];
-    }
-  }
+  strip_sum(parts, p0, p1, S, c, nk, acc);
   float* dst = out + static_cast<int64_t>(blockIdx.y) * S + c;
-  for (int k = 0; k < 4 && c + k < S; ++k) dst[k] = acc[k];
+  for (int k = 0; k < nk; ++k) dst[k] = acc[k];
 }
 
 __global__ void col_reduce_ordered_kernel(const float* __restrict__ parts,
@@ -157,23 +90,14 @@
                                           float* __restrict__ out) {
   const int c = (blockIdx.x * blockDim.x + threadIdx.x) * 4;
   const bool active = c < S;
+  const int nk = min(4, S - c);
   if (active) {
     const int p0 = blockIdx.y * chunk;
     const int p1 = min(p0 + chunk, nparts);
     float acc[4] = {};
-    for (int p = p0; p < p1; ++p) {
-      const float* src = parts + static_cast<int64_t>(p) * S + c;
-      if (c + 4 <= S) {
-        float v[4];
-        *reinterpret_cast<uint4*>(v) = *reinterpret_cast<const uint4*>(src);
-#pragma unroll
-        for (int k = 0; k < 4; ++k) acc[k] += v[k];
-      } else {
-        for (int k = 0; c + k < S; ++k) acc[k] += src[k];
-      }
-    }
+    strip_sum(parts, p0, p1, S, c, nk, acc);
     float* dst = tmp + static_cast<int64_t>(blockIdx.y) * S + c;
-    for (int k = 0; k < 4 && c + k < S; ++k) dst[k] = acc[k];
+    for (int k = 0; k < nk; ++k) dst[k] = acc[k];
   }
   __threadfence();
   __shared__ bool is_last;
@@ -183,30 +107,8 @@
   __syncthreads();
   if (!is_last || !active) return;
   __threadfence();
-  constexpr int kFoldBatch = 16;
-  const int ny = static_cast<int>(gridDim.y);
-  const int nk = min(4, S - c);
   float sum[4] = {};
-  for (int j0 = 0; j0 < ny; j0 += kFoldBatch) {
-    float v[kFoldBatch][4];
-#pragma unroll
-    for (int u = 0; u < kFoldBatch; ++u) {
-      const int j = min(j0 + u, ny - 1);
-      const float* src = tmp + static_cast<int64_t>(j) * S + c;
-      if (nk == 4) {
-        *reinterpret_cast<uint4*>(v[u]) =
-            *reinterpret_cast<const uint4*>(src);
-      } else {
-#pragma unroll
-        for (int k = 0; k < 4; ++k) v[u][k] = k < nk ? src[k] : 0.f;
-      }
-    }
-#pragma unroll
-    for (int u = 0; u < kFoldBatch; ++u)
-      if (j0 + u < ny) {
-        for (int k = 0; k < 4; ++k) sum[k] += v[u][k];
-      }
-  }
+  strip_sum(tmp, 0, static_cast<int>(gridDim.y), S, c, nk, sum);
   for (int k = 0; k < nk; ++k) out[c + k] = sum[k];
 }
 
@@ -236,31 +138,6 @@
                      reinterpret_cast<unsigned int*>(counters.data_ptr<int>()),
                      out.data_ptr<float>());
   return out;
-}
-
-torch::Tensor col_stats(torch::Tensor dy, torch::Tensor z,
-                        torch::Tensor dx_src, torch::Tensor mean,
-                        torch::Tensor rstd) {
-  const int rows = z.size(0), H = z.size(1);
-  const int rows_per_chunk = 16;
-  const int n_chunks = (rows + rows_per_chunk - 1) / rows_per_chunk;
-  const bool has_bias = dx_src.defined();
-  auto part = torch::empty({n_chunks, (has_bias ? 3 : 2) * H},
-                           z.options().dtype(torch::kFloat32));
-  auto stream = at::hip::getCurrentHIPStream();
-  DISPATCH_ROW_DTYPE(z.scalar_type(), "col_stats", [&] {
-    const int threads = tmin(256, ((H / kVec + 63) / 64) * 64);
-    dim3 grid((H / kVec + threads - 1) / threads, n_chunks);
-    by_flag(has_bias, [&](auto bias_c) {
-      hipLaunchKernelGGL(
-          (col_stats_kernel<scalar_t, kVec, decltype(bias_c)::value>), grid,
-          dim3(threads), 0, stream, dptr<scalar_t>(dy), dptr<scalar_t>(z),
-          has_bias ? dptr<scalar_t>(dx_src) : nullptr, mean.data_ptr<float>(),
-          rstd.data_ptr<float>(), part.data_ptr<float>(), rows, H,
-          rows_per_chunk);
-    });
-  });
-  return col_reduce_full(part);
 }
 
 std::vector<torch::Tensor> ln_fwd(torch::Tensor x, torch::Tensor gamma,
@@ -300,18 +177,14 @@
   auto gamma_f = gamma.contiguous().to(torch::kFloat32);
   auto dx = torch::empty_like(x);
   auto stream = at::hip::getCurrentHIPStream();
+  torch::Tensor part, none;
   DISPATCH_ROW_DTYPE(x.scalar_type(), "ln_bwd", [&] {
     TORCH_CHECK(H % kVec == 0, "ln_bwd: H must be a multiple of ", kVec);
-    launch_by_items("ln_bwd", H / kVec, [&](auto items_c, int threads) {
-      hipLaunchKernelGGL(
-          (ln_bwd_dx_kernel<scalar_t, kVec, decltype(items_c)::value>),
-          dim3(rows), dim3(threads), 0, stream, dptr<scalar_t>(dy),
-          dptr<scalar_t>(x), gamma_f.data_ptr<float>(),
-          mean.data_ptr<float>(), rstd.data_ptr<float>(), dptr<scalar_t>(dx),
-          rows, H);
-    });
+    part = ln_bwd_rows<scalar_t, kVec, false>("ln_bwd", dy, none, x, none,
+                                              gamma_f, mean, rstd, dx, none,
+                                              0.0, false, stream);
   });
-  auto dgb = col_stats(dy, x, torch::Tensor(), mean, rstd);
+  auto dgb = col_reduce_full(part);
   auto dgamma = dgb.narrow(0, 0, H);
   auto dbeta = dgb.narrow(0, H, H);
   if (gamma.scalar_type() != torch::kFloat32) {
diff --git a/csrc/ops/rowwise.h b/csrc/ops/rowwise.h
--- a/csrc/ops/rowwise.h
+++ b/csrc/ops/rowwise.h
@@ -2,6 +2,7 @@
 
 #include <torch/extension.h>
 
+#include <algorithm>
 #include <type_traits>
 
 #include "../common.h"
@@ -155,11 +156,12 @@
 }
 
 template <typename T>
-__device__ __forceinline__ void ln_bwd_elem(T x, T dy, const float* gamma,
+__device__ __forceinline__ void ln_bwd_elem(T x, float dy, float gamma,
                                             float mu, float rs, float& dw,
                                             float& xh, float& s1, float& s2) {
+#pragma clang fp contract(off)
   xh = (DTraits<T>::to_f32(x) - mu) * rs;
-  dw = DTraits<T>::to_f32(dy) * *gamma;
+  dw = dy * gamma;
   s1 += dw * xh;
   s2 += dw;
 }
@@ -173,7 +175,227 @@
 
 __device__ __forceinline__ float ln_bwd_dz(float dw, float xh, float rs,
                                            float s1, float s2) {
-  return rs * (dw - s2 - xh * s1);
-}
-
-}
+#pragma clang fp contract(off)
+  return rs * __builtin_fmaf(-xh, s1, dw - s2);
+}
+
+constexpr int kRowGroupThreads = 512;
+constexpr int kRowGroupBlocks = 512;
+constexpr int kRowGroupMinRows = 2;
+
+template <typename T, int VEC, int ITEMS, bool DROP, bool DY2>
+struct LnBwdRow {
+  T dy[ITEMS][VEC], x[ITEMS][VEC];
+  T dy2[DY2 ? ITEMS : 1][VEC];
+  uint8_t keep[DROP ? ITEMS : 1][VEC];
+  float mu, rs;
+};
+
+template <typename T, int VEC, int ITEMS, bool JUNCTION, bool TRAIN_DROP,
+          bool HAS_BIAS, bool HAS_DY2>
+__global__ void
+__launch_bounds__(ITEMS <= 2 ? kRowGroupThreads : 1024, ITEMS == 2 ? 2 : 4)
+ln_bwd_rows_kernel(
+    const T* __restrict__ dy, const T* __restrict__ dy2,
+    const T* __restrict__ x, const uint8_t* __restrict__ mask,
+    const float* __restrict__ gamma, const float* __restrict__ mean,
+    const float* __restrict__ rstd, T* __restrict__ dx,
+    T* __restrict__ dz_res, float* __restrict__ part, int rows, int H,
+    int rows_per_block, float p) {
+  static_assert(JUNCTION || !(TRAIN_DROP || HAS_BIAS || HAS_DY2), "");
+  constexpr bool kPipe = ITEMS * VEC <= 8;
+  constexpr int NSL = HAS_BIAS ? 3 : 2;
+  using Row = LnBwdRow<T, VEC, ITEMS, TRAIN_DROP, HAS_DY2>;
+  extern __shared__ float slab[];
+  __shared__ float red[2][kRowGroupThreads / WAVE_SIZE][32];
+  const int lanes = blockDim.y, y = threadIdx.y;
+  const int r_begin = blockIdx.x * rows_per_block;
+  const int r_end = min(r_begin + rows_per_block, rows);
+  const float keep_scale = TRAIN_DROP ? 1.0f / (1.0f - p) : 1.0f;
+
+  int cols[ITEMS];
+  float g[kPipe ? ITEMS : 1][VEC];
+#pragma unroll
+  for (int i = 0; i < ITEMS; ++i) {
+    cols[i] = (i * blockDim.x + threadIdx.x) * VEC;
+    if (kPipe && cols[i] < H) {
+#pragma unroll
+      for (int k = 0; k < VEC; ++k) g[i][k] = gamma[cols[i] + k];
+    }
+  }
+  auto load_row = [&](Row& r, int row) {
+    const int64_t base = static_cast<int64_t>(row) * H;
+    r.mu = mean[row];
+    r.rs = rstd[row];
+#pragma unroll
+    for (int i = 0; i < ITEMS; ++i) {
+      const int c = cols[i];
+      if (c < H) {
+        load_slice(dy + base + c, r.dy[i]);
+        if (HAS_DY2) load_slice(dy2 + base + c, r.dy2[i]);
+        load_slice(x + base + c, r.x[i]);
+        if (TRAIN_DROP) load_mask(mask + base + c, r.keep[i]);
+      }
+    }
+  };
+
+  float acc[NSL][ITEMS][VEC] = {};
+  Row cur, nxt;
+  int row = r_begin + y;
+  if (kPipe && row < r_end) load_row(cur, row);
+  for (int it = 0; r_begin + it * lanes < r_end; ++it, row += lanes) {
+    const bool valid = row < r_end;
+    if (kPipe) {
+      if (row + lanes < r_end) load_row(nxt, row + lanes);
+    } else if (valid) {
+      load_row(cur, row);
+    }
+    float dw[ITEMS][VEC], xh[ITEMS][VEC];
+    float s1 = 0.f, s2 = 0.f;
+    if (valid) {
+#pragma unroll
+      for (int i = 0; i < ITEMS; ++i) {
+        const int c = cols[i];
+        if (c < H) {
+#pragma unroll
+          for (int k = 0; k < VEC; ++k) {
+            float d = DTraits<T>::to_f32(cur.dy[i][k]);
+            if (HAS_DY2) d += DTraits<T>::to_f32(cur.dy2[i][k]);
+            const float gk = kPipe ? g[i][k] : gamma[c + k];
+            ln_bwd_elem(cur.x[i][k], d, gk, cur.mu, cur.rs, dw[i][k],
+                        xh[i][k], s1, s2);
+            acc[0][i][k] += d * xh[i][k];
+            acc[1][i][k] += d;
+          }
+        }
+      }
+    }
+    ln_bwd_row_means(s1, s2, H, red[it & 1][y]);
+    if (valid) {
+      const int64_t base = static_cast<int64_t>(row) * H;
+#pragma unroll
+      for (int i = 0; i < ITEMS; ++i) {
+        const int c = cols[i];
+        if (c < H) {
+          T dzo[VEC], dxo[VEC];
+#pragma unroll
+          for (int k = 0; k < VEC; ++k) {
+            const float dzk = ln_bwd_dz(dw[i][k], xh[i][k], cur.rs, s1, s2);
+            dzo[k] = DTraits<T>::from_f32(dzk);
+            if (JUNCTION) {
+              float dxk = dzk;
+              if (TRAIN_DROP) {
+                dxk = cur.keep[i][k] ? dzk * keep_scale : 0.f;
+                asm("" : "+v"(dxk));
+              }
+              dxo[k] = DTraits<T>::from_f32(dxk);
+              if (HAS_BIAS) acc[NSL - 1][i][k] += DTraits<T>::to_f32(dxo[k]);
+            }
+          }
+          if (JUNCTION) {
+            store_slice(dz_res + base + c, dzo);
+            store_slice(dx + base + c, dxo);
+          } else {
+            store_slice(dx + base + c, dzo);
+          }
+        }
+      }
+    }
+    if (kPipe) cur = nxt;
+  }
+
+  float* out = part + static_cast<int64_t>(blockIdx.x) * NSL * H;
+#pragma unroll
+  for (int sl = 0; sl < NSL; ++sl) {
+    if (lanes == 1) {
+#pragma unroll
+      for (int i = 0; i < ITEMS; ++i) {
+        if (cols[i] < H) {
+#pragma unroll
+          for (int k = 0; k < VEC; ++k)
+            out[sl * H + cols[i] + k] = acc[sl][i][k];
+        }
+      }
+      continue;
+    }
+    if (sl > 0) __syncthreads();
+#pragma unroll
+    for (int i = 0; i < ITEMS; ++i) {
+#pragma unroll
+      for (int k = 0; k < VEC; ++k)
+        slab[((y * ITEMS + i) * VEC + k) * blockDim.x + threadIdx.x] =
+            acc[sl][i][k];
+    }
+    __syncthreads();
+    if (y == sl % lanes) {
+#pragma unroll
+      for (int i = 0; i < ITEMS; ++i) {
+        if (cols[i] < H) {
+          float tot[VEC] = {};
+          for (int j = 0; j < lanes; ++j) {
+#pragma unroll
+            for (int k = 0; k < VEC; ++k)
+              tot[k] +=
+                  slab[((j * ITEMS + i) * VEC + k) * blockDim.x + threadIdx.x];
+          }
+#pragma unroll
+          for (int k = 0; k < VEC; ++k) out[sl * H + cols[i] + k] = tot[k];
+        }
+      }
+    }
+  }
+}
+
+template <typename T, int VEC, bool JUNCTION>
+inline torch::Tensor ln_bwd_rows(const char* op, const torch::Tensor& dy,
+                                 const torch::Tensor& dy2,
+                                 const torch::Tensor& x,
+                                 const torch::Tensor& mask,
+                                 const torch::Tensor& gamma_f,
+                                 const torch::Tensor& mean,
+                                 const torch::Tensor& rstd, torch::Tensor& dx,
+                                 torch::Tensor& dz_res, double p,
+                                 bool has_bias, hipStream_t stream) {
+  const int rows = x.size(0), H = x.size(1);
+  const int nsl = has_bias ? 3 : 2;
+  auto fopts = x.options().dtype(torch::kFloat32);
+  if (rows == 0) return torch::zeros({1, nsl * H}, fopts);
+  const bool train_drop = JUNCTION && p > 0.0;
+  const bool has_dy2 = dy2.defined();
+  torch::Tensor part;
+  launch_by_items(op, H / VEC, [&](auto items_c, int threads) {
+    constexpr int ITEMS = decltype(items_c)::value;
+    const int lanes =
+        threads >= kRowGroupThreads ? 1 : kRowGroupThreads / threads;
+    const int groups = (rows + lanes - 1) / lanes;
+    const int rows_per_lane = std::max(
+        kRowGroupMinRows, (groups + kRowGroupBlocks - 1) / kRowGroupBlocks);
+    const int rows_per_block = rows_per_lane * lanes;
+    const int nblocks = (rows + rows_per_block - 1) / rows_per_block;
+    part = torch::empty({nblocks, nsl * H}, fopts);
+    const size_t lds =
+        lanes > 1 ? sizeof(float) * lanes * threads * ITEMS * VEC : 0;
+    by_flag(train_drop, [&](auto train_c) {
+      by_flag(has_bias, [&](auto bias_c) {
+        by_flag(has_dy2, [&](auto dy2_c) {
+          constexpr bool kTrain = JUNCTION && decltype(train_c)::value;
+          constexpr bool kBias = JUNCTION && decltype(bias_c)::value;
+          constexpr bool kDy2 = JUNCTION && decltype(dy2_c)::value;
+          hipLaunchKernelGGL(
+              (ln_bwd_rows_kernel<T, VEC, ITEMS, JUNCTION, kTrain, kBias,
+                                  kDy2>),
+              dim3(nblocks), dim3(threads, lanes), lds, stream, dptr<T>(dy),
+              kDy2 ? dptr<T>(dy2) : nullptr, dptr<T>(x),
+              kTrain ? mask.data_ptr<uint8_t>() : nullptr,
+              gamma_f.data_ptr<float>(), mean.data_ptr<float>(),
+              rstd.data_ptr<float>(), dptr<T>(dx),
+              JUNCTION ? dptr<T>(dz_res) : nullptr, part.data_ptr<float>(),
+              rows, H, rows_per_block, static_cast<float>(p));
+        });
+      });
+    });
+  });
+  return part;
+}
+
+}
```

Measured after the change: 2637 seq/s (median of 6 runs). 1.05x the previous value.
